# nivihelen99/NetFlow

Measured on AMD Instinct MI355X. Metric: device-resident payload GB/s checksummed, batched packets, 1/2/4/8 MI355X, higher is better.
Workload: dtype u16 one's-complement (u8 frames, u32 word sums); 1 GPU; C1: 1M x 1500 B IPv4+UDP, device-resident; packets_per_gpu=1048576, frame_align=128, frame_bytes_per_gpu=1572864000, parallelism=independent shards x1

## Files before the change

include/nfcs.h:

```cpp
#ifndef NFCS_H
#define NFCS_H

#include <stddef.h>
#include <stdint.h>

#ifdef __cplusplus
extern "C" {
#endif

#if defined(__GNUC__)
#define NFCS_API __attribute__((visibility("default")))
#else
#define NFCS_API
#endif

#define NFCS_ABI_VERSION 2


typedef struct nfcs_desc {
    uint32_t off16;
    uint32_t len;
} nfcs_desc;

typedef struct nfcs_patch {
    uint16_t ip_off;
    uint16_t l4_off;
    uint8_t ip[2];
    uint8_t l4[2];
} nfcs_patch;

#define NFCS_PATCH_NONE 0xFFFFu

enum {
    NFCS_ST_NONE = 0,
    NFCS_ST_V4 = 1,
    NFCS_ST_V4_TCP = 2,
    NFCS_ST_V4_UDP = 3,
    NFCS_ST_V4_ICMP = 4,
    NFCS_ST_V4_L4SKIP = 5,
    NFCS_ST_V6 = 6,
    NFCS_ST_V6_TCP = 7,
    NFCS_ST_V6_UDP = 8,
    NFCS_ST_V6_L4SKIP = 9,
    NFCS_ST_NO_ROUTE = 11,
    NFCS_ST_NOT_IPV4 = 12,
    NFCS_ST_TTL_EXPIRED = 13,
    NFCS_ST_OOB = 14,
    NFCS_ST_BAD_DESC = 15,
    NFCS_ST_VLAN_FAIL = 16,
    NFCS_ST_FLAG_VLAN = 0x20,
    NFCS_ST_FLAG_OVERLAP = 0x40,
    NFCS_ST_FLAG_FWD = 0x80
};

enum {
    NFCS_OK = 0,
    NFCS_EINVAL = -1,
    NFCS_EHIP = -2,
    NFCS_ENOMEM = -3,
    NFCS_ENODEV = -4
};

enum {
    NFCS_CFG_C0_64B_V4 = 0,
    NFCS_CFG_C1_1500B_UDP = 1,
    NFCS_CFG_C2_9000B_TCP = 2,
    NFCS_CFG_C3_MIXED = 3
};

typedef struct nfcs_ctx nfcs_ctx;

NFCS_API int nfcs_abi_version(void);
NFCS_API const char* nfcs_strerror(int err);
NFCS_API int nfcs_last_hip_error(void);


NFCS_API int nfcs_ctx_create(int device, nfcs_ctx** out);
NFCS_API int nfcs_ctx_destroy(nfcs_ctx* ctx);
NFCS_API void* nfcs_ctx_stream(nfcs_ctx* ctx);
NFCS_API int nfcs_ctx_set_slot_bytes(nfcs_ctx* ctx, uint32_t bytes);
NFCS_API int nfcs_ctx_launch_footprint(nfcs_ctx* ctx, uint64_t arena_bytes, const nfcs_desc* d_desc,
                                       uint32_t n, uint64_t* mean);
NFCS_API int nfcs_ctx_host_numa(nfcs_ctx* ctx, int* node, int* local);


NFCS_API int nfcs_update_device(nfcs_ctx* ctx, uint8_t* d_arena, uint64_t arena_bytes,
                                const nfcs_desc* d_desc, uint32_t n, uint8_t* d_status,
                                nfcs_patch* d_patch, void* stream);

#define NFCS_HOST_ZERO_COPY_AUTO_BYTES (32u << 20)
#define NFCS_HOST_PATCH_ONLY 1u
#define NFCS_HOST_ZERO_COPY 2u
#define NFCS_HOST_FRAMES 4u
NFCS_API int nfcs_update_host(nfcs_ctx* ctx, uint8_t* h_arena, uint64_t arena_bytes,
                              const nfcs_desc* h_desc, uint32_t n, uint8_t* h_status,
                              uint32_t flags);

#define NFCS_FRAME_RELEVANT_BYTES 131072u
NFCS_API int nfcs_update_host_frames(nfcs_ctx* ctx, uint8_t* const* frames, const uint32_t* lens, uint32_t n,
                                     uint8_t* h_status, uint32_t flags);


typedef struct nfcs_nexthop {
    uint8_t dst_mac[6];
    uint8_t src_mac[6];
} nfcs_nexthop;
#define NFCS_NH_NONE 0xFFFFFFFFu

NFCS_API int nfcs_l3_forward_device(nfcs_ctx* ctx, uint8_t* d_arena, uint64_t arena_bytes,
                                    const nfcs_desc* d_desc, const uint32_t* d_nh, uint32_t n,
                                    const nfcs_nexthop* d_table, uint32_t table_n,
                                    uint8_t* d_status, void* stream);



enum {
    NFCS_RT_FORWARD = 0,
    NFCS_RT_BAD_DESC = 1,
    NFCS_RT_NOT_IPV4 = 2,
    NFCS_RT_LOCAL = 3,
    NFCS_RT_TTL_EXPIRED = 4,
    NFCS_RT_NO_ROUTE = 5,
    NFCS_RT_ARP_MISS = 6,
    NFCS_RT_NO_IF_MAC = 7
};
#define NFCS_IF_NONE 0xFFFFFFFFu

typedef struct nfcs_fib_route {
    uint32_t network;
    uint32_t mask;
    uint32_t next_hop_ip;
    uint32_t egress_if;
} nfcs_fib_route;
typedef struct nfcs_fib_arp {
    uint32_t ip;
    uint8_t mac[6];
    uint8_t pad[2];
} nfcs_fib_arp;
typedef struct nfcs_fib_if_mac {
    uint32_t egress_if;
    uint8_t mac[6];
    uint8_t pad[2];
} nfcs_fib_if_mac;

#define NFCS_FIB_MAX_ROUTES 4096u

typedef struct nfcs_fib nfcs_fib;
NFCS_API int nfcs_fib_create(nfcs_fib** out);
NFCS_API int nfcs_fib_destroy(nfcs_fib* fib);
NFCS_API int nfcs_fib_set_routes(nfcs_fib* fib, const nfcs_fib_route* routes, uint32_t n);
NFCS_API int nfcs_fib_set_arp(nfcs_fib* fib, const nfcs_fib_arp* arp, uint32_t n);
NFCS_API int nfcs_fib_set_if_macs(nfcs_fib* fib, const nfcs_fib_if_mac* if_macs, uint32_t n);
NFCS_API int nfcs_fib_set_local_ips(nfcs_fib* fib, const uint32_t* ips, uint32_t n);
NFCS_API int nfcs_fib_commit(nfcs_fib* fib);
NFCS_API int nfcs_fib_upload(nfcs_ctx* ctx, nfcs_fib* fib);
NFCS_API int nfcs_fib_nexthops(const nfcs_fib* fib, const nfcs_nexthop** d_table, uint32_t* table_n);
NFCS_API int nfcs_fib_nexthops_host(const nfcs_fib* fib, nfcs_nexthop* out, uint32_t cap, uint32_t* table_n);
NFCS_API int nfcs_fib_lookup_host(const nfcs_fib* fib, uint32_t dst_ip, uint32_t ttl, uint32_t* verdict,
                                  uint32_t* nh, uint32_t* egress_if);

NFCS_API int nfcs_route_lookup_device(nfcs_ctx* ctx, const nfcs_fib* fib, const uint8_t* d_arena,
                                      uint64_t arena_bytes, const nfcs_desc* d_desc, uint32_t n,
                                      uint32_t* d_nh, uint32_t* d_egress_if, uint8_t* d_verdict,
                                      void* stream);

// ... 284 lines not shown
#define NFCS_ACL_LIST_NONE 0xFFFFFFFFu
#define NFCS_ACL_NO_PORT 4u
typedef struct nfcs_aclset nfcs_aclset;
NFCS_API int nfcs_aclset_create(nfcs_aclset** out);
NFCS_API int nfcs_aclset_destroy(nfcs_aclset* set);
NFCS_API int nfcs_aclset_set_list(nfcs_aclset* set, uint32_t list_id, const nfcs_acl_rule* rules, uint32_t n);
NFCS_API int nfcs_aclset_remove_list(nfcs_aclset* set, uint32_t list_id);
NFCS_API int nfcs_aclset_bind_port(nfcs_aclset* set, uint32_t port_id, uint32_t list_id);
NFCS_API int nfcs_aclset_clear(nfcs_aclset* set);
NFCS_API int nfcs_aclset_commit(nfcs_aclset* set);
NFCS_API int nfcs_aclset_upload(nfcs_ctx* ctx, nfcs_aclset* set);
NFCS_API int nfcs_aclset_info(const nfcs_aclset* set, uint32_t* ports, uint32_t* lists, uint32_t* rules_padded);
NFCS_API int nfcs_aclset_eval_host(const nfcs_aclset* set, uint32_t port, const uint8_t* frame, uint32_t len,
                                   uint32_t* action, uint32_t* rule_index, uint32_t* redirect_port);

NFCS_API int nfcs_egress_acl_device(nfcs_ctx* ctx, const nfcs_aclset* set, const uint8_t* d_arena,
                                    uint64_t arena_bytes, const nfcs_desc* d_desc, uint32_t n, uint32_t* d_port,
                                    uint8_t* d_action, uint32_t* d_rule, uint32_t* d_redirect,
                                    uint32_t* d_denied_pkts, uint64_t* d_denied_bytes, void* stream);
NFCS_API int nfcs_egress_acl_host(const nfcs_aclset* set, const uint8_t* arena, uint64_t arena_bytes,
                                  const nfcs_desc* desc, uint32_t n, uint32_t* port, uint8_t* action,
                                  uint32_t* rule, uint32_t* redirect, uint32_t* denied_pkts,
                                  uint64_t* denied_bytes);


enum { NFCS_SCHED_STRICT_PRIORITY = 0, NFCS_SCHED_WRR = 1, NFCS_SCHED_DRR = 2 };
typedef struct nfcs_txq nfcs_txq;

NFCS_API int nfcs_txq_create(nfcs_ctx* ctx, const nfcs_egress* eg, nfcs_txq** out);
NFCS_API int nfcs_txq_destroy(nfcs_txq* txq);
NFCS_API int nfcs_txq_set_scheduler(nfcs_txq* txq, uint32_t port_id, uint32_t sched);
NFCS_API int nfcs_txq_reset(nfcs_txq* txq);
NFCS_API int nfcs_txq_info(const nfcs_txq* txq, uint32_t* ports, uint32_t* keys, uint64_t* ring_slots);
NFCS_API int nfcs_txq_state_device(nfcs_txq* txq, uint32_t* head, uint8_t* last, void* stream);
NFCS_API int nfcs_txq_state_host(const nfcs_txq* txq, uint32_t* head, uint8_t* last);

NFCS_API int nfcs_txq_append_device(nfcs_ctx* ctx, nfcs_txq* txq, const uint32_t* d_order,
                                    const uint32_t* d_key_start, const uint32_t* d_depth, const uint64_t* d_handle,
                                    const nfcs_desc* d_desc, uint32_t n, void* stream);
NFCS_API int nfcs_txq_append_host(nfcs_txq* txq, const uint32_t* order, const uint32_t* key_start,
                                  const uint32_t* depth, const uint64_t* handle, const nfcs_desc* desc, uint32_t n);

NFCS_API int nfcs_txq_dequeue_device(nfcs_ctx* ctx, nfcs_txq* txq, const uint32_t* d_budget, uint32_t budget_all,
                                     uint32_t* d_depth, uint64_t* d_tx, uint32_t tx_cap, uint8_t* d_tx_queue,
                                     uint32_t* d_tx_start, uint32_t* d_dequeued, void* stream);
NFCS_API int nfcs_txq_dequeue_host(nfcs_txq* txq, const uint32_t* budget, uint32_t budget_all, uint32_t* depth,
                                   uint64_t* tx, uint32_t tx_cap, uint8_t* tx_queue, uint32_t* tx_start,
                                   uint32_t* dequeued);
NFCS_API int nfcs_txq_closed_form_host(uint32_t sched, uint32_t num_queues, uint32_t last, const uint32_t* depth,
                                       uint32_t budget, uint32_t* take, uint32_t* new_last, uint8_t* seq,
                                       uint32_t seq_cap);


typedef struct nfcs_flow_key {
    uint32_t hash;
    uint16_t vlan_id;
    uint16_t ethertype;
    uint8_t src_mac[6];
    uint8_t dst_mac[6];
    uint8_t protocol;
    uint8_t is_ipv6;
    uint16_t src_port;
    uint16_t dst_port;
    uint8_t reserved[6];
    uint8_t src_ip[16];
    uint8_t dst_ip[16];
} nfcs_flow_key;

NFCS_API int nfcs_flow_keys_device(nfcs_ctx* ctx, const uint8_t* d_arena, uint64_t arena_bytes,
                                   const nfcs_desc* d_desc, uint32_t n, nfcs_flow_key* d_keys,
                                   uint32_t* d_hash, void* stream);


NFCS_API int nfcs_shard_bytes(const nfcs_desc* h_desc, uint32_t n, uint32_t parts, uint32_t* bounds);


NFCS_API int nfcs_layout_config(int config, uint64_t seed, uint64_t first_index, uint32_t n,
                                uint32_t align, nfcs_desc* h_desc, uint64_t* arena_bytes);

NFCS_API int nfcs_gen_config_device(nfcs_ctx* ctx, int config, uint64_t seed,
                                    uint64_t first_index, uint32_t n, uint8_t* d_arena,
                                    uint64_t arena_bytes, const nfcs_desc* d_desc, void* stream);

NFCS_API int nfcs_digest_device(nfcs_ctx* ctx, const uint8_t* d_arena, uint64_t arena_bytes,
                                const nfcs_desc* d_desc, uint32_t n, uint64_t first_index,
                                uint64_t* h_digest, void* stream);

NFCS_API int nfcs_device_alloc(nfcs_ctx* ctx, size_t bytes, void** out);
NFCS_API int nfcs_device_free(nfcs_ctx* ctx, void* p);
NFCS_API int nfcs_host_alloc(nfcs_ctx* ctx, size_t bytes, void** out);
NFCS_API int nfcs_host_free(nfcs_ctx* ctx, void* p);
NFCS_API int nfcs_memcpy_h2d(nfcs_ctx* ctx, void* dst, const void* src, size_t bytes);
NFCS_API int nfcs_memcpy_d2h(nfcs_ctx* ctx, void* dst, const void* src, size_t bytes);
NFCS_API int nfcs_stream_sync(nfcs_ctx* ctx, void* stream);

NFCS_API int nfcs_time_update_device(nfcs_ctx* ctx, uint8_t* d_arena, uint64_t arena_bytes,
                                     const nfcs_desc* d_desc, uint32_t n, uint8_t* d_status,
                                     int iters, void* stream, float* ms);
NFCS_API int nfcs_time_update_batches(nfcs_ctx* ctx, uint32_t batches, uint8_t* const* d_arenas,
                                      const uint64_t* arena_bytes, const nfcs_desc* const* d_descs,
                                      uint32_t n, int iters, void* stream, float* ms);
NFCS_API int nfcs_time_flow_keys_device(nfcs_ctx* ctx, const uint8_t* d_arena, uint64_t arena_bytes,
                                        const nfcs_desc* d_desc, uint32_t n, nfcs_flow_key* d_keys,
                                        uint32_t* d_hash, int iters, void* stream, float* ms);
NFCS_API int nfcs_time_l3_forward_device(nfcs_ctx* ctx, uint8_t* d_arena, uint64_t arena_bytes,
                                         const nfcs_desc* d_desc, const uint32_t* d_nh,
                                         uint32_t n, const nfcs_nexthop* d_table, uint32_t table_n,
                                         uint8_t* d_status, int iters, void* stream, float* ms);

NFCS_API int nfcs_time_stream_read(nfcs_ctx* ctx, const uint8_t* d_buf, uint64_t bytes, int form,
                                   int iters, void* stream, float* ms);
NFCS_API int nfcs_time_frames_read(nfcs_ctx* ctx, const uint8_t* d_arena, uint64_t arena_bytes,
                                   const nfcs_desc* d_desc, uint32_t n, int iters, void* stream, float* ms);
NFCS_API int nfcs_time_vlan_device(nfcs_ctx* ctx, uint8_t* d_arena, uint64_t arena_bytes,
                                   nfcs_desc* d_desc, uint32_t n, uint32_t op_all,
                                   uint32_t op_alt, uint32_t cap_all, uint8_t* d_status, int iters,
                                   void* stream, float* ms);

#ifdef __cplusplus
}
#endif
#endif
```

netflow_amd/__init__.py:

```python
from __future__ import annotations

import ctypes
import os
import subprocess

import numpy as np

HERE = os.path.dirname(os.path.abspath(__file__))
ROOT = os.path.dirname(HERE)
LIB_PATH = os.environ.get("NFCS_LIB") or os.path.join(HERE, "libnfcs.so")
HEADER = os.path.join(ROOT, "include", "nfcs.h")
SOURCES = [os.path.join(HERE, "csrc", "nfcs_kernels.hip"), os.path.join(HERE, "csrc", "nfcs_api.hip")]

DESC_DTYPE = np.dtype([("off16", "<u4"), ("len", "<u4")])
PATCH_DTYPE = np.dtype([("ip_off", "<u2"), ("l4_off", "<u2"), ("ip", "u1", (2,)), ("l4", "u1", (2,))])

ST_NONE, ST_V4, ST_V4_TCP, ST_V4_UDP, ST_V4_ICMP, ST_V4_L4SKIP = 0, 1, 2, 3, 4, 5
ST_V6, ST_V6_TCP, ST_V6_UDP, ST_V6_L4SKIP, ST_OOB, ST_BAD_DESC = 6, 7, 8, 9, 14, 15
ST_FLAG_OVERLAP = 0x40
ST_NO_ROUTE, ST_NOT_IPV4, ST_TTL_EXPIRED, ST_FLAG_FWD = 11, 12, 13, 0x80
NH_NONE = 0xFFFFFFFF
ST_VLAN_FAIL, ST_FLAG_VLAN = 16, 0x20
VLAN_NOP, VLAN_PUSH, VLAN_POP = 0, 0x40000000, 0x80000000


def vlan_push_op(vid: int, prio: int = 0) -> int:
    return VLAN_PUSH | ((prio & 7) << 13) | (vid & 0xFFF)

RT_FORWARD, RT_BAD_DESC, RT_NOT_IPV4, RT_LOCAL, RT_TTL_EXPIRED, RT_NO_ROUTE, RT_ARP_MISS, RT_NO_IF_MAC = range(8)
IF_NONE = 0xFFFFFFFF
FIB_MAX_ROUTES = 4096
FIB_ROUTE_DTYPE = np.dtype([("network", "<u4"), ("mask", "<u4"), ("next_hop_ip", "<u4"), ("egress_if", "<u4")])
FIB_ARP_DTYPE = np.dtype([("ip", "<u4"), ("mac", "u1", (6,)), ("pad", "u1", (2,))])
FIB_IF_MAC_DTYPE = np.dtype([("egress_if", "<u4"), ("mac", "u1", (6,)), ("pad", "u1", (2,))])

ACL_PERMIT, ACL_DENY, ACL_REDIRECT, ACL_BAD_DESC = range(4)
ACL_NO_MATCH = 0xFFFFFFFF
ACL_MAX_RULES = 512
ACL_GROUP = 4
(ACL_F_SRC_MAC, ACL_F_DST_MAC, ACL_F_VLAN_ID, ACL_F_ETHERTYPE, ACL_F_SRC_IP, ACL_F_DST_IP, ACL_F_PROTOCOL,
 ACL_F_SRC_PORT, ACL_F_DST_PORT) = (1 << k for k in range(9))
ACL_RULE_DTYPE = np.dtype([("fields", "<u4"), ("rule_id", "<u4"), ("src_mac", "u1", (6,)), ("dst_mac", "u1", (6,)),
                           ("vlan_id", "<u2"), ("ethertype", "<u2"), ("src_ip", "<u4"), ("dst_ip", "<u4"),
                           ("src_ip_mask", "<u4"), ("dst_ip_mask", "<u4"), ("src_port", "<u2"), ("dst_port", "<u2"),
                           ("protocol", "u1"), ("action", "u1"), ("pad", "u1", (2,)), ("redirect_port", "<u4")])
assert ACL_RULE_DTYPE.itemsize == 52
ACL_NO_PORT = 4
ACL_LIST_NONE = 0xFFFFFFFF
ACLSET_MAX_LISTS = 128

(L2_FORWARD, L2_BAD_DESC, L2_SKIP, L2_NO_ETH, L2_FLOOD, L2_DROP_SAME_PORT, L2_DROP_LINK_DOWN, L2_DROP_STP,
 L2_DROP_VLAN) = range(9)
L2_LEARN_NONE, L2_LEARN_NEW, L2_LEARN_REFRESH, L2_LEARN_MOVED = range(4)
L2_ACCESS, L2_TRUNK, L2_HYBRID = range(3)
FDB_MAX_ENTRIES = 1 << 20
L2_MAX_PORTS = 1024
FDB_ENTRY_DTYPE = np.dtype([("mac", "u1", (6,)), ("vlan_id", "<u2"), ("port", "<u4"), ("is_static", "u1"),
                            ("pad", "u1", (3,))])
L2_PORT_DTYPE = np.dtype([("port_id", "<u4"), ("link_up", "u1"), ("stp_forwarding", "u1"), ("has_vlan_config", "u1"),
                          ("type", "u1"), ("native_vlan", "<u2"), ("pad", "<u2")])
assert FDB_ENTRY_DTYPE.itemsize == 16 and L2_PORT_DTYPE.itemsize == 12

FLOOD_TILE_PKTS = 1024
ITEM_NONE = 0xFFFFFFFF
FLOOD_TOTALS_DTYPE = np.dtype([("items", "<u4"), ("items_needed", "<u4"), ("copies", "<u4"), ("flooded", "<u4"),
                               ("copy_bytes", "<u8"), ("copy_bytes_needed", "<u8")])
assert FLOOD_TOTALS_DTYPE.itemsize == 32

ICMP_TILE_PKTS = 1024
(ICMP_ST_NONE, ICMP_ST_ECHO_REPLY, ICMP_ST_TIME_EXCEEDED, ICMP_ST_UNREACHABLE, ICMP_ST_TO_CPU, ICMP_ST_IGNORED,
 ICMP_ST_NO_LOCAL_MAC, ICMP_ST_SRC_NO_ROUTE, ICMP_ST_SRC_NO_IF_IP, ICMP_ST_SRC_ARP_MISS, ICMP_ST_SRC_NO_IF_MAC,
 ICMP_ST_PORT_DOWN, ICMP_ST_OOB, ICMP_ST_TOO_LONG, ICMP_ST_OVERFLOW) = range(15)
ICMP_LOCAL_DTYPE = np.dtype([("ip", "<u4"), ("mac", "u1", (6,)), ("pad", "u1", (2,))])
ICMP_IF_IP_DTYPE = np.dtype([("egress_if", "<u4"), ("ip", "<u4")])
ICMP_TOTALS_DTYPE = np.dtype([("messages", "<u4"), ("messages_needed", "<u4"), ("echo_replies", "<u4"),
                              ("errors", "<u4"), ("msg_bytes", "<u8"), ("msg_bytes_needed", "<u8")])
assert ICMP_LOCAL_DTYPE.itemsize == 12 and ICMP_IF_IP_DTYPE.itemsize == 8 and ICMP_TOTALS_DTYPE.itemsize == 32

QOS_MAX_QUEUES = 8
QUEUE_NONE = 0xFF
EGRESS_TILE_PKTS = 1024
EQ_ENQUEUED, EQ_SKIP, EQ_DROP_NO_CONFIG, EQ_DROP_FULL, EQ_BAD_QUEUE = range(5)
EGRESS_PORT_DTYPE = np.dtype([("port_id", "<u4"), ("has_vlan_config", "u1"), ("type", "u1"), ("tag_native", "u1"),
                              ("has_qos", "u1"), ("native_vlan", "<u2"), ("num_queues", "u1"), ("pad", "u1"),
                              ("max_queue_depth", "<u4")])
assert EGRESS_PORT_DTYPE.itemsize == 16
SCHED_STRICT_PRIORITY, SCHED_WRR, SCHED_DRR = range(3)

NEXTHOP_DTYPE = np.dtype([("dst_mac", "u1", (6,)), ("src_mac", "u1", (6,))])
FLOW_KEY_DTYPE = np.dtype([("hash", "<u4"), ("vlan_id", "<u2"), ("ethertype", "<u2"),
                           ("src_mac", "u1", (6,)), ("dst_mac", "u1", (6,)), ("protocol", "u1"),
                           ("is_ipv6", "u1"), ("src_port", "<u2"), ("dst_port", "<u2"),
                           ("reserved", "u1", (6,)), ("src_ip", "u1", (16,)), ("dst_ip", "u1", (16,))])
assert FLOW_KEY_DTYPE.itemsize == 64
CFG_C0, CFG_C1, CFG_C2, CFG_C3 = 0, 1, 2, 3
HOST_PATCH_ONLY, HOST_ZERO_COPY, HOST_FRAMES = 1, 2, 4
PATCH_NONE = 0xFFFF


class NfcsError(RuntimeError):
    pass


KERNARG_PRELOAD = ["-mllvm", "-amdgpu-kernarg-preload-count=8"]


def build(verbose: bool = False) -> str:
    out = os.path.join(HERE, "libnfcs.so")
    cmd = ["hipcc", "--offload-arch=gfx950", "-O3", "-fPIC", "-shared", "-std=c++17", *KERNARG_PRELOAD,
           "-I" + os.path.join(ROOT, "include"), "-I" + os.path.join(HERE, "csrc"), *SOURCES, "-o", out]
    if verbose:
        print(" ".join(cmd))
    subprocess.run(cmd, check=True)
    return out


ABI_VERSION = 2
_lib = None
_vp = ctypes.c_void_p
_u32 = ctypes.c_uint32
_u64 = ctypes.c_uint64


def _declare(L):
    sig = {
        "nfcs_abi_version": ([], ctypes.c_int),
        "nfcs_strerror": ([ctypes.c_int], ctypes.c_char_p),
        "nfcs_last_hip_error": ([], ctypes.c_int),
        "nfcs_ctx_create": ([ctypes.c_int, ctypes.POINTER(_vp)], ctypes.c_int),
        "nfcs_ctx_destroy": ([_vp], ctypes.c_int),
        "nfcs_ctx_stream": ([_vp], _vp),
        "nfcs_ctx_set_slot_bytes": ([_vp, ctypes.c_uint32], ctypes.c_int),
        "nfcs_ctx_launch_footprint": ([_vp, _u64, _vp, _u32, ctypes.POINTER(_u64)], ctypes.c_int),
        "nfcs_update_device": ([_vp, _vp, _u64, _vp, _u32, _vp, _vp, _vp], ctypes.c_int),
        "nfcs_update_host": ([_vp, _vp, _u64, _vp, _u32, _vp, _u32], ctypes.c_int),
        "nfcs_update_host_frames": ([_vp, _vp, _vp, _u32, _vp, _u32], ctypes.c_int),
        "nfcs_layout_config": ([ctypes.c_int, _u64, _u64, _u32, _u32, _vp, ctypes.POINTER(_u64)], ctypes.c_int),
        "nfcs_shard_bytes": ([_vp, _u32, _u32, _vp], ctypes.c_int),
        "nfcs_ctx_host_numa": ([_vp, ctypes.POINTER(ctypes.c_int), ctypes.POINTER(ctypes.c_int)], ctypes.c_int),
        "nfcs_gen_config_device": ([_vp, ctypes.c_int, _u64, _u64, _u32, _vp, _u64, _vp, _vp], ctypes.c_int),
        "nfcs_digest_device": ([_vp, _vp, _u64, _vp, _u32, _u64, ctypes.POINTER(_u64), _vp], ctypes.c_int),
        "nfcs_device_alloc": ([_vp, ctypes.c_size_t, ctypes.POINTER(_vp)], ctypes.c_int),
        "nfcs_device_free": ([_vp, _vp], ctypes.c_int),
        "nfcs_host_alloc": ([_vp, ctypes.c_size_t, ctypes.POINTER(_vp)], ctypes.c_int),
        "nfcs_host_free": ([_vp, _vp], ctypes.c_int),
        "nfcs_memcpy_h2d": ([_vp, _vp, _vp, ctypes.c_size_t], ctypes.c_int),
        "nfcs_memcpy_d2h": ([_vp, _vp, _vp, ctypes.c_size_t], ctypes.c_int),
        "nfcs_stream_sync": ([_vp, _vp], ctypes.c_int),
        "nfcs_time_update_device": ([_vp, _vp, _u64, _vp, _u32, _vp, ctypes.c_int, _vp,
                                     ctypes.POINTER(ctypes.c_float)], ctypes.c_int),
        "nfcs_time_update_batches": ([_vp, _u32, _vp, _vp, _vp, _u32, ctypes.c_int, _vp,
                                      ctypes.POINTER(ctypes.c_float)], ctypes.c_int),
        "nfcs_l3_forward_device": ([_vp, _vp, _u64, _vp, _vp, _u32, _vp, _u32, _vp, _vp],
                                   ctypes.c_int),
        "nfcs_vlan_device": ([_vp, _vp, _u64, _vp, _u32, _vp, _u32, _vp, _u32, _vp, _vp],
                             ctypes.c_int),
        "nfcs_time_vlan_device": ([_vp, _vp, _u64, _vp, _u32, _u32, _u32, _u32, _vp, ctypes.c_int,
                                   _vp, ctypes.POINTER(ctypes.c_float)], ctypes.c_int),
        "nfcs_flow_keys_device": ([_vp, _vp, _u64, _vp, _u32, _vp, _vp, _vp], ctypes.c_int),
        "nfcs_time_stream_read": ([_vp, _vp, _u64, ctypes.c_int, ctypes.c_int, _vp, _vp], ctypes.c_int),
        "nfcs_time_frames_read": ([_vp, _vp, _u64, _vp, _u32, ctypes.c_int, _vp, _vp], ctypes.c_int),
        "nfcs_time_flow_keys_device": ([_vp, _vp, _u64, _vp, _u32, _vp, _vp, ctypes.c_int, _vp,
                                        ctypes.POINTER(ctypes.c_float)], ctypes.c_int),
        "nfcs_time_l3_forward_device": ([_vp, _vp, _u64, _vp, _vp, _u32, _vp, _u32, _vp,
                                         ctypes.c_int, _vp, ctypes.POINTER(ctypes.c_float)],
                                        ctypes.c_int),
        "nfcs_fib_create": ([ctypes.POINTER(_vp)], ctypes.c_int),
        "nfcs_fib_destroy": ([_vp], ctypes.c_int),
        "nfcs_fib_set_routes": ([_vp, _vp, _u32], ctypes.c_int),
        "nfcs_fib_set_arp": ([_vp, _vp, _u32], ctypes.c_int),
        "nfcs_fib_set_if_macs": ([_vp, _vp, _u32], ctypes.c_int),
        "nfcs_fib_set_local_ips": ([_vp, _vp, _u32], ctypes.c_int),
        "nfcs_fib_commit": ([_vp], ctypes.c_int),
        "nfcs_fib_upload": ([_vp, _vp], ctypes.c_int),
        "nfcs_fib_nexthops": ([_vp, ctypes.POINTER(_vp), ctypes.POINTER(_u32)], ctypes.c_int),
        "nfcs_fib_nexthops_host": ([_vp, _vp, _u32, ctypes.POINTER(_u32)], ctypes.c_int),
        "nfcs_fib_lookup_host": ([_vp, _u32, _u32, ctypes.POINTER(_u32), ctypes.POINTER(_u32),
                                  ctypes.POINTER(_u32)], ctypes.c_int),
        "nfcs_route_lookup_device": ([_vp, _vp, _vp, _u64, _vp, _u32, _vp, _vp, _vp, _vp], ctypes.c_int),
        "nfcs_acl_create": ([ctypes.POINTER(_vp)], ctypes.c_int),
        "nfcs_acl_destroy": ([_vp], ctypes.c_int),
        "nfcs_acl_set_rules": ([_vp, _vp, _u32], ctypes.c_int),
        "nfcs_acl_commit": ([_vp], ctypes.c_int),
        "nfcs_acl_upload": ([_vp, _vp], ctypes.c_int),
        "nfcs_acl_eval_host": ([_vp, _vp, _u32, ctypes.POINTER(_u32), ctypes.POINTER(_u32),
                                ctypes.POINTER(_u32)], ctypes.c_int),
        "nfcs_acl_eval_device": ([_vp, _vp, _vp, _u64, _vp, _u32, _vp, _vp, _vp, _vp, _vp], ctypes.c_int),
        "nfcs_fdb_create": ([ctypes.POINTER(_vp)], ctypes.c_int),
        "nfcs_fdb_destroy": ([_vp], ctypes.c_int),
        "nfcs_fdb_set_entries": ([_vp, _vp, _u32], ctypes.c_int),
        "nfcs_fdb_set_port": ([_vp, _vp, _vp, _u32], ctypes.c_int),
        "nfcs_fdb_clear_ports": ([_vp], ctypes.c_int),
        "nfcs_fdb_commit": ([_vp], ctypes.c_int),
        "nfcs_fdb_upload": ([_vp, _vp], ctypes.c_int),
        "nfcs_fdb_stats": ([_vp] + [ctypes.POINTER(_u32)] * 4, ctypes.c_int),
        "nfcs_fdb_lookup_host": ([_vp, _u32, _vp, _u32] + [ctypes.POINTER(_u32)] * 4, ctypes.c_int),
        "nfcs_fdb_flood_ports_host": ([_vp, _u32, _u32, _u32, _vp, _u32, ctypes.POINTER(_u32)], ctypes.c_int),
        "nfcs_l2_lookup_device": ([_vp, _vp, _u32, _vp, _u64, _vp, _u32, _vp, _vp, _vp, _vp, _vp, _vp],
                                  ctypes.c_int),
        "nfcs_flood_expand_device": ([_vp, _vp, _u32, _u32, _vp, _u64, _u64, _u32, _vp, _u32] + [_vp] * 5 + [_u32] +
                                     [_vp] * 5, ctypes.c_int),
        "nfcs_flood_expand_host": ([_vp, _u32, _u32, _u64, _u64, _u32, _vp, _u32] + [_vp] * 5 + [_u32] + [_vp] * 4,
                                   ctypes.c_int),
        "nfcs_icmp_create": ([ctypes.POINTER(_vp)], ctypes.c_int),
        "nfcs_icmp_destroy": ([_vp], ctypes.c_int),
        "nfcs_icmp_set_local": ([_vp, _vp, _u32], ctypes.c_int),
        "nfcs_icmp_set_if_ips": ([_vp, _vp, _u32], ctypes.c_int),
        "nfcs_icmp_set_ports_up": ([_vp, _vp, _u32, _u32], ctypes.c_int),
        "nfcs_icmp_commit": ([_vp], ctypes.c_int),
        "nfcs_icmp_upload": ([_vp, _vp], ctypes.c_int),
        "nfcs_fib_resolve_host": ([_vp, _u32, ctypes.POINTER(_u32), ctypes.POINTER(_u32), ctypes.POINTER(_u32)],
                                  ctypes.c_int),
        "nfcs_icmp_respond_device": ([_vp, _vp, _vp, _u32, _vp, _u64, _u64, _u32, _vp, _u32, _vp, _vp, _u32] +
                                     [_vp] * 6, ctypes.c_int),
        "nfcs_icmp_respond_host": ([_vp, _vp, _u32, _vp, _u64, _u64, _u32, _vp, _u32, _vp, _vp, _u32] + [_vp] * 5,
                                   ctypes.c_int),
        "nfcs_egress_create": ([ctypes.POINTER(_vp)], ctypes.c_int),
        "nfcs_egress_destroy": ([_vp], ctypes.c_int),
        "nfcs_egress_set_port": ([_vp, _vp], ctypes.c_int),
        "nfcs_egress_clear_ports": ([_vp], ctypes.c_int),
        "nfcs_egress_commit": ([_vp], ctypes.c_int),
        "nfcs_egress_upload": ([_vp, _vp], ctypes.c_int),
        "nfcs_egress_keys": ([_vp, ctypes.POINTER(_u32), ctypes.POINTER(_u32)], ctypes.c_int),
# ... 611 lines not shown
    cap = int(min(int(depth.sum(dtype=np.uint64)), budget)) if want_seq else 0
    seq = np.full(cap, QUEUE_NONE, np.uint8)
    _check(lib().nfcs_txq_closed_form_host(int(sched), nq, int(last), depth.ctypes.data if nq else None, int(budget),
                                           take.ctypes.data if nq else None, ctypes.byref(new_last),
                                           seq.ctypes.data if cap else None, cap), "nfcs_txq_closed_form_host")
    return take, int(new_last.value), seq if want_seq else None


class DeviceBuffer:

    def __init__(self, engine: "Engine", nbytes: int):
        self.engine = engine
        self.nbytes = int(nbytes)
        p = _vp()
        _check(lib().nfcs_device_alloc(engine.ctx, max(self.nbytes, 16), ctypes.byref(p)), "device_alloc")
        self.ptr = p.value

    def upload(self, a: np.ndarray, offset: int = 0):
        a = np.ascontiguousarray(a)
        if offset < 0 or offset + a.nbytes > self.nbytes:
            raise NfcsError(f"upload of {a.nbytes} B at {offset} past a {self.nbytes}-byte buffer")
        if a.nbytes:
            _check(lib().nfcs_memcpy_h2d(self.engine.ctx, self.ptr + offset, a.ctypes.data, a.nbytes), "h2d")
        return self

    def download(self, dtype=np.uint8, count: int | None = None, offset: int = 0) -> np.ndarray:
        dtype = np.dtype(dtype)
        count = (self.nbytes - offset) // dtype.itemsize if count is None else count
        if offset < 0 or offset + count * dtype.itemsize > self.nbytes:
            raise NfcsError(f"download of {count} x {dtype} at {offset} past a {self.nbytes}-byte buffer")
        out = np.empty(count, dtype=dtype)
        if out.nbytes:
            _check(lib().nfcs_memcpy_d2h(self.engine.ctx, out.ctypes.data, self.ptr + offset, out.nbytes), "d2h")
        return out

    def free(self):
        if self.ptr:
            lib().nfcs_device_free(self.engine.ctx, self.ptr)
            self.ptr = None

    def __del__(self):
        try:
            self.free()
        except Exception:
            pass


class Engine:

    def __init__(self, device: int = 0):
        self.device = device
        self._pinned = {}
        c = _vp()
        _check(lib().nfcs_ctx_create(device, ctypes.byref(c)), f"nfcs_ctx_create({device})")
        self.ctx = c.value

    def close(self):
        if getattr(self, "ctx", None):
            for p in list(self._pinned):
                lib().nfcs_host_free(self.ctx, p)
            self._pinned.clear()
            lib().nfcs_ctx_destroy(self.ctx)
            self.ctx = None

    def __enter__(self):
        return self

    def __exit__(self, *a):
        self.close()

    @property
    def stream(self) -> int:
        return lib().nfcs_ctx_stream(self.ctx)

    def set_slot_bytes(self, nbytes: int):
        _check(lib().nfcs_ctx_set_slot_bytes(self.ctx, int(nbytes)), "set_slot_bytes")

    def launch_footprint(self, arena_bytes: int, desc, n: int) -> int:
        m = _u64()
        p = desc.ptr if isinstance(desc, DeviceBuffer) else int(desc)
        _check(lib().nfcs_ctx_launch_footprint(self.ctx, arena_bytes, p, n, ctypes.byref(m)), "launch_footprint")
        return int(m.value)

    def host_numa(self) -> tuple[int, bool]:
        node, local = ctypes.c_int(), ctypes.c_int()
        _check(lib().nfcs_ctx_host_numa(self.ctx, ctypes.byref(node), ctypes.byref(local)), "host_numa")
        return node.value, bool(local.value)

    def alloc(self, nbytes: int) -> DeviceBuffer:
        return DeviceBuffer(self, nbytes)

    def host_array(self, nbytes: int) -> np.ndarray:
        p = _vp()
        size = max(int(nbytes), 16)
        _check(lib().nfcs_host_alloc(self.ctx, size, ctypes.byref(p)), "host_alloc")
        self._pinned[p.value] = size
        return np.ctypeslib.as_array((ctypes.c_uint8 * size).from_address(p.value))[:nbytes]

    def host_free(self, arr: np.ndarray):
        p = arr.__array_interface__["data"][0]
        if self._pinned.pop(p, None) is None:
            raise NfcsError("host_free: not a live host_array of this engine")
        _check(lib().nfcs_host_free(self.ctx, p), "host_free")

    def sync(self, stream=None):
        _check(lib().nfcs_stream_sync(self.ctx, stream), "stream_sync")

    def update_device(self, arena: DeviceBuffer | int, arena_bytes: int, desc: DeviceBuffer | int,
                      n: int, status=None, patch=None, stream=None):
        ptr = lambda b: None if b is None else (b.ptr if isinstance(b, DeviceBuffer) else int(b))
        _check(lib().nfcs_update_device(self.ctx, ptr(arena), arena_bytes, ptr(desc), n,
                                        ptr(status), ptr(patch), stream), "nfcs_update_device")

    def update_host(self, arena: np.ndarray, desc: np.ndarray, want_status: bool = True,
                    mode: str = "patch") -> np.ndarray | None:
        flags = {"patch": 0, "frames": HOST_FRAMES, "zero_copy": HOST_ZERO_COPY}[mode]
        assert arena.dtype == np.uint8 and arena.flags.c_contiguous
        desc = np.ascontiguousarray(desc, dtype=DESC_DTYPE)
        n = len(desc)
        status = np.zeros(n, dtype=np.uint8) if want_status else None
        _check(lib().nfcs_update_host(self.ctx, arena.ctypes.data, arena.nbytes,
                                      desc.ctypes.data if n else None, n,
                                      status.ctypes.data if want_status and n else None,
                                      flags), "nfcs_update_host")
        return status

    def update_host_frames(self, buf: np.ndarray, offsets: np.ndarray, lens: np.ndarray,
                           want_status: bool = True) -> np.ndarray | None:
        assert buf.dtype == np.uint8 and buf.flags.c_contiguous
        offsets = np.asarray(offsets, dtype=np.int64)
        lens = np.ascontiguousarray(lens, dtype=np.uint32)
        n = len(lens)
        assert len(offsets) == n and (n == 0 or int((offsets + lens.astype(np.int64)).max()) <= buf.nbytes)
        ptrs = np.where(offsets < 0, 0, np.uint64(buf.ctypes.data) + offsets.astype(np.uint64)).astype(np.uint64)
        status = np.zeros(n, dtype=np.uint8) if want_status else None
        _check(lib().nfcs_update_host_frames(self.ctx, ptrs.ctypes.data if n else None,
                                             lens.ctypes.data if n else None, n,
                                             status.ctypes.data if want_status and n else None, 0),
               "nfcs_update_host_frames")
        return status

    def l3_forward_device(self, arena, arena_bytes: int, desc, nh, n: int, table, table_n: int,
                          status=None, stream=None):
        ptr = lambda b: None if b is None else (b.ptr if isinstance(b, DeviceBuffer) else int(b))
        _check(lib().nfcs_l3_forward_device(self.ctx, ptr(arena), arena_bytes, ptr(desc), ptr(nh), n,
                                            ptr(table), table_n, ptr(status), stream),
               "nfcs_l3_forward_device")

    def route_lookup_device(self, fib: Fib, arena, arena_bytes: int, desc, n: int, nh, egress_if=None,
                            verdict=None, stream=None):
        ptr = lambda b: None if b is None else (b.ptr if isinstance(b, DeviceBuffer) else int(b))
        _check(lib().nfcs_route_lookup_device(self.ctx, fib.ptr, ptr(arena), arena_bytes, ptr(desc), n, ptr(nh),
                                              ptr(egress_if), ptr(verdict), stream), "nfcs_route_lookup_device")

    def acl_eval_device(self, acl: Acl, arena, arena_bytes: int, desc, n: int, action, rule=None, redirect=None,
                        nh=None, stream=None):
        ptr = lambda b: None if b is None else (b.ptr if isinstance(b, DeviceBuffer) else int(b))
        _check(lib().nfcs_acl_eval_device(self.ctx, acl.ptr, ptr(arena), arena_bytes, ptr(desc), n, ptr(action),
                                          ptr(rule), ptr(redirect), ptr(nh), stream), "nfcs_acl_eval_device")

    def l2_lookup_device(self, fdb: "Fdb", ingress_port: int, arena, arena_bytes: int, desc, n: int, egress_port,
                         rt_verdict=None, verdict=None, vlan=None, learn=None, stream=None):
        ptr = lambda b: None if b is None else (b.ptr if isinstance(b, DeviceBuffer) else int(b))
        _check(lib().nfcs_l2_lookup_device(self.ctx, fdb.ptr, int(ingress_port), ptr(arena), arena_bytes, ptr(desc), n,
                                           ptr(rt_verdict), ptr(egress_port), ptr(verdict), ptr(vlan), ptr(learn),
                                           stream), "nfcs_l2_lookup_device")
# ... 49 lines not shown
        ptr = lambda b: None if b is None else (b.ptr if isinstance(b, DeviceBuffer) else int(b))
        _check(lib().nfcs_txq_dequeue_device(self.ctx, txq.ptr, ptr(budget), int(budget_all), ptr(depth), ptr(tx),
                                             int(tx_cap), ptr(tx_queue), ptr(tx_start), ptr(dequeued), stream),
               "nfcs_txq_dequeue_device")

    def vlan_device(self, arena, arena_bytes: int, desc, n: int, ops=None, op_all: int = 0,
                    caps=None, cap_all: int = 0, status=None, stream=None):
        ptr = lambda b: None if b is None else (b.ptr if isinstance(b, DeviceBuffer) else int(b))
        _check(lib().nfcs_vlan_device(self.ctx, ptr(arena), arena_bytes, ptr(desc), n, ptr(ops),
                                      op_all, ptr(caps), cap_all, ptr(status), stream),
               "nfcs_vlan_device")

    def time_vlan_device(self, arena, arena_bytes, desc, n, op_all, op_alt, cap_all, iters,
                         status=None, stream=None) -> float:
        ms = ctypes.c_float()
        ptr = lambda b: None if b is None else (b.ptr if isinstance(b, DeviceBuffer) else int(b))
        _check(lib().nfcs_time_vlan_device(self.ctx, ptr(arena), arena_bytes, ptr(desc), n, op_all,
                                           op_alt, cap_all, ptr(status), iters, stream,
                                           ctypes.byref(ms)), "time_vlan_device")
        return float(ms.value)

    def flow_keys_device(self, arena, arena_bytes: int, desc, n: int, keys=None, hashes=None,
                         stream=None):
        ptr = lambda b: None if b is None else (b.ptr if isinstance(b, DeviceBuffer) else int(b))
        _check(lib().nfcs_flow_keys_device(self.ctx, ptr(arena), arena_bytes, ptr(desc), n, ptr(keys),
                                           ptr(hashes), stream), "nfcs_flow_keys_device")

    def time_flow_keys_device(self, arena, arena_bytes, desc, n, keys, hashes, iters,
                              stream=None) -> float:
        ms = ctypes.c_float()
        ptr = lambda b: None if b is None else (b.ptr if isinstance(b, DeviceBuffer) else int(b))
        _check(lib().nfcs_time_flow_keys_device(self.ctx, ptr(arena), arena_bytes, ptr(desc), n,
                                                ptr(keys), ptr(hashes), iters, stream,
                                                ctypes.byref(ms)), "time_flow_keys_device")
        return float(ms.value)

    def time_stream_read(self, buf, nbytes, iters, form=0, stream=None) -> float:
        ms = ctypes.c_float()
        p = buf.ptr if isinstance(buf, DeviceBuffer) else int(buf)
        _check(lib().nfcs_time_stream_read(self.ctx, p, nbytes & ~15, form, iters, stream,
                                           ctypes.byref(ms)), "time_stream_read")
        return float(ms.value)

    def time_frames_read(self, arena, arena_bytes, desc, n, iters, stream=None) -> float:
        ms = ctypes.c_float()
        p = lambda b: b.ptr if isinstance(b, DeviceBuffer) else int(b)
        _check(lib().nfcs_time_frames_read(self.ctx, p(arena), arena_bytes, p(desc), n, iters, stream,
                                           ctypes.byref(ms)), "time_frames_read")
        return float(ms.value)

    def time_l3_forward_device(self, arena, arena_bytes, desc, nh, n, table, table_n, iters,
                               status=None, stream=None) -> float:
        ms = ctypes.c_float()
        ptr = lambda b: None if b is None else (b.ptr if isinstance(b, DeviceBuffer) else int(b))
        _check(lib().nfcs_time_l3_forward_device(self.ctx, ptr(arena), arena_bytes, ptr(desc),
                                                 ptr(nh), n, ptr(table), table_n, ptr(status),
                                                 iters, stream, ctypes.byref(ms)),
               "time_l3_forward_device")
        return float(ms.value)

    def time_update_device(self, arena, arena_bytes, desc, n, iters, status=None, stream=None) -> float:
        ms = ctypes.c_float()
        _check(lib().nfcs_time_update_device(self.ctx, arena.ptr, arena_bytes, desc.ptr, n,
                                             None if status is None else status.ptr, iters, stream,
                                             ctypes.byref(ms)), "time_update_device")
        return float(ms.value)

    def time_update_batches(self, batches, n, iters, stream=None) -> float:
        k = len(batches)
        p = lambda b: b.ptr if isinstance(b, DeviceBuffer) else int(b)
        arenas = (_vp * k)(*[p(a) for a, _, _ in batches])
        sizes = (_u64 * k)(*[int(nb) for _, nb, _ in batches])
        descs = (_vp * k)(*[p(d) for _, _, d in batches])
        ms = ctypes.c_float()
        _check(lib().nfcs_time_update_batches(self.ctx, k, arenas, sizes, descs, n, iters, stream,
                                              ctypes.byref(ms)), "time_update_batches")
        return float(ms.value)

    def gen_config_device(self, config: int, seed: int, first: int, n: int,
                          arena: DeviceBuffer, arena_bytes: int, desc: DeviceBuffer, stream=None):
        _check(lib().nfcs_gen_config_device(self.ctx, config, seed, first, n, arena.ptr, arena_bytes,
                                            desc.ptr, stream), "gen_config_device")

    def digest_device(self, arena: DeviceBuffer, arena_bytes: int, desc: DeviceBuffer, n: int,
                      first: int = 0, stream=None) -> int:
        out = _u64()
        _check(lib().nfcs_digest_device(self.ctx, arena.ptr, arena_bytes, desc.ptr, n, first,
                                        ctypes.byref(out), stream), "digest_device")
        return int(out.value)

    def config_batch(self, config: int, seed: int, first: int, n: int, align: int = 16):
        hdesc, nbytes = layout_config(config, seed, first, n, align)
        d_desc = self.alloc(max(hdesc.nbytes, 16)).upload(hdesc)
        d_arena = self.alloc(max(nbytes, 16))
        self.gen_config_device(config, seed, first, n, d_arena, nbytes, d_desc)
        self.sync()
        return d_arena, nbytes, d_desc, hdesc
```

netflow_amd/csrc/nfcs_api.hip:

```cpp
#include <pthread.h>
#include <sched.h>
#include <stdio.h>
#include <stdlib.h>
#include <string.h>
#include <sys/mman.h>
#include <sys/syscall.h>
#include <unistd.h>

#include <algorithm>
#include <chrono>
#include <condition_variable>
#include <mutex>
#include <new>
#include <thread>
#include <vector>

#include "nfcs_internal.h"

struct HostBlock {
    void* p = nullptr;
    size_t bytes = 0;
    bool mapped = false;
};

class Workers {
public:
    ~Workers() { stop(); }
    void start(int n, const cpu_set_t* cpus) noexcept {
        for (int i = 0; i < n; ++i) {
            try {
                th_.emplace_back([this, cpus] { loop(cpus); });
            } catch (...) {
                break;
            }
        }
    }
    void stop() noexcept {
        {
            std::lock_guard<std::mutex> l(mu_);
            quit_ = true;
        }
        cv_.notify_all();
        for (auto& t : th_) t.join();
        th_.clear();
        quit_ = false;
    }
    int size() const { return (int)th_.size(); }
    template <class F>
    void run(int k, const F& fn) noexcept {
        if (k <= 1 || th_.empty()) {
            for (int i = 0; i < k; ++i) fn(i);
            return;
        }
        run_erased(k, [](const void* f, int i) { (*(const F*)f)(i); }, &fn);
    }

private:
    void run_erased(int k, void (*call)(const void*, int), const void* fn) noexcept {
        std::unique_lock<std::mutex> l(mu_);
        call_ = call;
        job_ = fn;
        parts_ = k;
        next_ = 0;
        pending_ = k;
        ++gen_;
        cv_.notify_all();
        take(l);
        done_.wait(l, [&] { return pending_ == 0; });
        job_ = nullptr;
    }
    void take(std::unique_lock<std::mutex>& l) {
        while (next_ < parts_) {
            const int i = next_++;
            void (*const call)(const void*, int) = call_;
            const void* const f = job_;
            l.unlock();
            call(f, i);
            l.lock();
            if (--pending_ == 0) done_.notify_all();
        }
    }
    void loop(const cpu_set_t* cpus) {
        if (cpus) (void)pthread_setaffinity_np(pthread_self(), sizeof(cpu_set_t), cpus);
        std::unique_lock<std::mutex> l(mu_);
        uint64_t seen = 0;
        for (;;) {
            cv_.wait(l, [&] { return quit_ || (gen_ != seen && next_ < parts_); });
            if (quit_) return;
            take(l);
            seen = gen_;
        }
    }
    std::vector<std::thread> th_;
    std::mutex mu_;
    std::condition_variable cv_, done_;
    void (*call_)(const void*, int) = nullptr;
    const void* job_ = nullptr;
    int parts_ = 0, next_ = 0, pending_ = 0;
    uint64_t gen_ = 0;
    bool quit_ = false;
};

struct nfcs_ctx {
    nfcs::DevInfo di;
    int numa_node = -1;
    bool numa_local = false;
    bool have_cpus = false;
    cpu_set_t node_cpus;
    HostBlock hb[2];
    hipStream_t stream = nullptr;
    static constexpr int kSlots = 2;
    static constexpr size_t kStageBytes = size_t(64) << 20;
    bool host_ready = false;
    hipStream_t hs[kSlots] = {nullptr, nullptr};
    hipEvent_t done[kSlots] = {nullptr, nullptr};
    hipEvent_t staged[kSlots] = {nullptr, nullptr};
    size_t stage_bytes = 0;
    uint32_t stage_pkts = 0;
    int copy_threads = 8;
    Workers workers;
    uint8_t* d_arena[kSlots] = {nullptr, nullptr};
    nfcs_desc* d_desc[kSlots] = {nullptr, nullptr};
    uint8_t* d_status[kSlots] = {nullptr, nullptr};
    nfcs_patch* d_patch[kSlots] = {nullptr, nullptr};
    uint64_t* done_host = nullptr;
    uint64_t* done_dev = nullptr;
    uint64_t* done_ctr = nullptr;
    uint64_t done_base[kSlots] = {0, 0};
    int slot_wait[kSlots] = {0, 0};
    uint8_t* z_block[kSlots] = {nullptr, nullptr};
    uint8_t* h_arena[kSlots] = {nullptr, nullptr};
    nfcs_desc* h_desc[kSlots] = {nullptr, nullptr};
    uint8_t* h_status[kSlots] = {nullptr, nullptr};
    nfcs_patch* h_patch[kSlots] = {nullptr, nullptr};
    uint64_t* d_digest = nullptr;
    hipEvent_t ev0 = nullptr, ev1 = nullptr;
    nfcs_patch* ws = nullptr;
    size_t ws_cap = 0;
    hipEvent_t ws_ev = nullptr;
    hipStream_t ws_stream = nullptr;
    bool ws_used = false;
    bool ws_own = false;
    uint32_t* eq_ws = nullptr;
    uint64_t eq_cap = 0;
    hipEvent_t eq_ev = nullptr;
    hipStream_t eq_stream = nullptr;
    bool eq_used = false;
    bool eq_own = false;
    uint32_t slot_bytes = 0;
    static constexpr int kObsSlots = 8;
    uint64_t* obs_host = nullptr;
    uint64_t* obs_dev = nullptr;
    struct ObsBurst { const void* desc; uint32_t n; uint64_t bytes; uint32_t gen; uint64_t used; };
    ObsBurst obs_burst[kObsSlots] = {};
    uint32_t obs_gen = 0;
    uint64_t obs_clock = 0;
};

namespace {

thread_local int g_last_hip = 0;

hipError_t wait_ws_user(nfcs_ctx* c, hipStream_t st) {
    if (c->ws_own) {
        hipError_t e = hipEventRecord(c->ws_ev, c->stream);
        if (e != hipSuccess) return e;
    }
    return st ? hipStreamWaitEvent(st, c->ws_ev, 0) : hipEventSynchronize(c->ws_ev);
}

hipError_t acquire_ws(nfcs_ctx* c, size_t n, hipStream_t st) {
    if (n > c->ws_cap) {
        if (c->ws_used) {
            hipError_t e = wait_ws_user(c, nullptr);
            if (e != hipSuccess) return e;
        }
        if (c->ws) (void)hipFree(c->ws);
        c->ws = nullptr;
        c->ws_cap = 0;
        c->ws_used = false;
        const size_t cap = n < (1u << 20) ? (1u << 20) : n;
        hipError_t e = hipMalloc(&c->ws, cap * sizeof(nfcs_patch));
        if (e != hipSuccess) return e;
        c->ws_cap = cap;
    } else if (c->ws_used && c->ws_stream != st) {
        hipError_t e = wait_ws_user(c, st);
        if (e != hipSuccess) return e;
    }
    return hipSuccess;
}
hipError_t release_ws(nfcs_ctx* c, hipStream_t st) {
    c->ws_stream = st;
    c->ws_used = true;
    c->ws_own = st == c->stream;
    return c->ws_own ? hipSuccess : hipEventRecord(c->ws_ev, st);
}

hipError_t wait_eq_user(nfcs_ctx* c, hipStream_t st) {
    if (c->eq_own) {
        hipError_t e = hipEventRecord(c->eq_ev, c->stream);
        if (e != hipSuccess) return e;
    }
    return st ? hipStreamWaitEvent(st, c->eq_ev, 0) : hipEventSynchronize(c->eq_ev);
}
hipError_t acquire_eq(nfcs_ctx* c, uint64_t words, hipStream_t st) {
    if (words > c->eq_cap) {
        if (c->eq_used) {
            hipError_t e = wait_eq_user(c, nullptr);
            if (e != hipSuccess) return e;
        }
        if (c->eq_ws) (void)hipFree(c->eq_ws);
        c->eq_ws = nullptr;
        c->eq_cap = 0;
        c->eq_used = false;
        const uint64_t cap = words < (1u << 18) ? (1u << 18) : words;
        if (cap > (uint64_t)SIZE_MAX / sizeof(uint32_t)) return hipErrorOutOfMemory;
        hipError_t e = hipMalloc(&c->eq_ws, (size_t)cap * sizeof(uint32_t));
        if (e != hipSuccess) {
            c->eq_ws = nullptr;
            (void)hipGetLastError();
            return hipErrorOutOfMemory;
        }
        c->eq_cap = cap;
    } else if (c->eq_used && c->eq_stream != st) {
        hipError_t e = wait_eq_user(c, st);
        if (e != hipSuccess) return e;
    }
    return hipSuccess;
}
hipError_t release_eq(nfcs_ctx* c, hipStream_t st) {
    c->eq_stream = st;
    c->eq_used = true;
    c->eq_own = st == c->stream;
    return c->eq_own ? hipSuccess : hipEventRecord(c->eq_ev, st);
}

int hip_fail(hipError_t e) {
    g_last_hip = (int)e;
    return NFCS_EHIP;
// ... 377 lines not shown
        } else {
            event_wait(c, s);
            e = hipMemcpyAsync(c->d_desc[s], c->h_desc[s], (size_t)m * sizeof(nfcs_desc),
                               hipMemcpyHostToDevice, st);
            if (e == hipSuccess)
                e = nfcs::launch_update(c->di, d_arena, arena_bytes, c->d_desc[s], m, 0u,
                                        h_status ? c->d_status[s] : nullptr, nullptr, nullptr,
                                        nfcs::kUpdateInline, st, shape);
            if (e == hipSuccess && h_status)
                e = hipMemcpyAsync(c->h_status[s], c->d_status[s], m, hipMemcpyDeviceToHost, st);
        }
        if (e == hipSuccess) e = hipEventRecord(c->done[s], st);
        if (e != hipSuccess) {
            (void)hipStreamSynchronize(st);
            break;
        }
        first[s] = i;
        cnt[s] = m;
        i += m;
    }
    finish(s);
    finish(s ^ 1);
    if (e != hipSuccess) return hip_fail(e);
    return NFCS_OK;
}

struct Shape { uint64_t mean; nfcs::ObsReq obs; uint32_t bits = 0; };
int find_burst(const nfcs_ctx* c, uint64_t arena_bytes, const nfcs_desc* d_desc, uint32_t n) {
    for (int k = 0; k < nfcs_ctx::kObsSlots; ++k) {
        const nfcs_ctx::ObsBurst& b = c->obs_burst[k];
        if (b.gen && b.desc == d_desc && b.n == n && b.bytes == arena_bytes) return k;
    }
    return -1;
}
bool sampled_estimate(uint64_t est, bool mid = false) {
    return mid || est >= nfcs::kSmallMeanBytes || est < nfcs::kTinyMeanBytes;
}
struct ShapeRule { uint64_t mix_mean; bool ring_rows8; bool bimodal_rows8; bool packed_rows8; };
constexpr ShapeRule kUpdateRule = {nfcs::kTinyMixMeanBytes, true, false, false};
constexpr ShapeRule kFwdRule = {nfcs::kTinyMixMeanBytes, true, true, true};
constexpr ShapeRule kVlanRule = {nfcs::kVlanMixMeanBytes, false, false, false};
Shape peek_shape(const nfcs_ctx* c, uint64_t arena_bytes, const nfcs_desc* d_desc, uint32_t n, int* slot,
                 const ShapeRule& rule = kUpdateRule) {
    *slot = -1;
    if (c->slot_bytes) return {c->slot_bytes, {}};
    if (n == 0) return {arena_bytes, {}};
    const uint64_t est = arena_bytes / n;
    if (!sampled_estimate(est, rule.packed_rows8) || !c->obs_host) return {est, {}};
    const int k = find_burst(c, arena_bytes, d_desc, n);
    if (k < 0) return {est, {}};
    *slot = k;
    const uint64_t o = __atomic_load_n(c->obs_host + k, __ATOMIC_RELAXED);
    const uint32_t gen = c->obs_burst[k].gen;
    const nfcs::ObsReq req = {c->obs_dev + k, ((uint64_t)gen << 32) | n};
    if ((uint32_t)(o >> 32) != gen || !((uint32_t)o & nfcs::kObsPresent)) return {est, req};
    uint64_t mean = std::min<uint64_t>((uint32_t)o & nfcs::kObsMeanMask, est);
    const bool bimodal = rule.bimodal_rows8 && (((uint32_t)o >> nfcs::kObsMidShift) & 7u) < nfcs::kObsMidMin8;
    if (mean < nfcs::kTinyMeanBytes && mean >= rule.mix_mean && !bimodal &&
        (((uint32_t)o >> nfcs::kObsLongShift) & 0x1FFu) > nfcs::kTinyLongMax)
        mean = nfcs::kTinyMeanBytes;
    const uint32_t bits = (uint32_t)o & (nfcs::kObsUnaligned | nfcs::kObsMixed);
    if (rule.ring_rows8 && !bits && (est >= nfcs::kSmallMeanBytes || rule.packed_rows8) &&
        mean >= nfcs::kTinyMeanBytes && mean < nfcs::kSmallMeanBytes)
        mean = nfcs::kTinyMeanBytes - 1;
    return {mean, req, bits};
}
Shape launch_shape(nfcs_ctx* c, uint64_t arena_bytes, const nfcs_desc* d_desc, uint32_t n,
                   const ShapeRule& rule = kUpdateRule) {
    int k = -1;
    Shape sh = peek_shape(c, arena_bytes, d_desc, n, &k, rule);
    if (sh.obs.slot == nullptr && k < 0 && !c->slot_bytes && n && c->obs_host &&
        sampled_estimate(arena_bytes / n, rule.packed_rows8)) {
        k = 0;
        for (int j = 1; j < nfcs_ctx::kObsSlots; ++j)
            if (c->obs_burst[j].used < c->obs_burst[k].used) k = j;
        if (++c->obs_gen == 0) c->obs_gen = 1;
        c->obs_burst[k] = {d_desc, n, arena_bytes, c->obs_gen, 0};
        sh.obs = {c->obs_dev + k, ((uint64_t)c->obs_gen << 32) | n};
    }
    if (k >= 0) c->obs_burst[k].used = ++c->obs_clock;
    return sh;
}

int update_device(nfcs_ctx* c, uint8_t* d_arena, uint64_t arena_bytes, const nfcs_desc* d_desc,
                  uint32_t n, uint8_t* d_status, nfcs_patch* d_patch, hipStream_t st) {
    if (!d_patch) NFCS_HIP(acquire_ws(c, n, st));
    const Shape sh = launch_shape(c, arena_bytes, d_desc, n);
    NFCS_HIP(nfcs::launch_update(c->di, d_arena, arena_bytes, d_desc, n, 0u, d_status, d_patch,
                                 d_patch ? nullptr : c->ws, nfcs::kUpdateAuto, st, sh.mean, sh.obs));
    if (!d_patch) NFCS_HIP(release_ws(c, st));
    return NFCS_OK;
}

int l3_forward_device(nfcs_ctx* c, uint8_t* d_arena, uint64_t arena_bytes, const nfcs_desc* d_desc,
                      const uint32_t* d_nh, uint32_t n, const nfcs_nexthop* d_table, uint32_t table_n,
                      uint8_t* d_status, hipStream_t st) {
    const bool dfr = n > nfcs::kFwdDeferAbovePackets;
    if (dfr) NFCS_HIP(acquire_ws(c, nfcs::kSubBatchPackets, st));
    const Shape sh = launch_shape(c, arena_bytes, d_desc, n, kFwdRule);
    NFCS_HIP(nfcs::launch_l3_forward(c->di, d_arena, arena_bytes, d_desc, d_nh, n, d_table, table_n,
                                     d_status, dfr ? c->ws : nullptr, st, sh.mean, sh.obs));
    if (dfr) NFCS_HIP(release_ws(c, st));
    return NFCS_OK;
}

}

extern "C" {

NFCS_API int nfcs_abi_version(void) { return NFCS_ABI_VERSION; }

NFCS_API const char* nfcs_strerror(int err) {
    switch (err) {
    case NFCS_OK: return "ok";
    case NFCS_EINVAL: return "invalid argument";
    case NFCS_EHIP: return "HIP runtime error";
    case NFCS_ENOMEM: return "out of memory";
    case NFCS_ENODEV: return "no gfx950 device";
    default: return "unknown error";
    }
}

NFCS_API int nfcs_last_hip_error(void) { return g_last_hip; }

NFCS_API int nfcs_ctx_create(int device, nfcs_ctx** out) {
    if (!out) return NFCS_EINVAL;
    *out = nullptr;
    int ndev = 0;
    if (hipGetDeviceCount(&ndev) != hipSuccess || device < 0 || device >= ndev) {
        (void)hipGetLastError();
        return NFCS_ENODEV;
    }
    DeviceGuard dg_(device);
    if (dg_.err != hipSuccess) return hip_fail(dg_.err);
    hipDeviceProp_t prop;
    NFCS_HIP(hipGetDeviceProperties(&prop, device));
    if (strncmp(prop.gcnArchName, "gfx950", 6) != 0) return NFCS_ENODEV;
    nfcs_ctx* c = new (std::nothrow) nfcs_ctx();
    if (!c) return NFCS_ENOMEM;
    c->di.device = device;
    c->di.cus = prop.multiProcessorCount;
    strncpy(c->di.arch, prop.gcnArchName, sizeof(c->di.arch) - 1);
    hipError_t e = hipStreamCreateWithFlags(&c->stream, hipStreamNonBlocking);
    if (e == hipSuccess) e = hipMalloc(&c->d_digest, sizeof(uint64_t));
    if (e == hipSuccess) e = hipEventCreateWithFlags(&c->ws_ev, hipEventDisableTiming);
    if (e == hipSuccess) e = hipEventCreateWithFlags(&c->eq_ev, hipEventDisableTiming);
    if (e == hipSuccess) e = hipEventCreate(&c->ev0);
    if (e == hipSuccess) e = hipEventCreate(&c->ev1);
    if (e == hipSuccess) e = hipHostMalloc((void**)&c->obs_host, nfcs_ctx::kObsSlots * sizeof(uint64_t), hipHostMallocMapped);
    if (e == hipSuccess) {
        for (int k = 0; k < nfcs_ctx::kObsSlots; ++k) c->obs_host[k] = 0;
        e = hipHostGetDevicePointer((void**)&c->obs_dev, c->obs_host, 0);
    }
    if (e != hipSuccess) {
        nfcs_ctx_destroy(c);
        return hip_fail(e);
    }
    *out = c;
    return NFCS_OK;
}

NFCS_API int nfcs_ctx_destroy(nfcs_ctx* c) {
    if (!c) return NFCS_OK;
    DeviceGuard dg_(c->di.device);
    if (c->stream) (void)hipStreamSynchronize(c->stream);
    if (c->ws_used && !c->ws_own && c->ws_ev) (void)hipEventSynchronize(c->ws_ev);
    if (c->eq_used && !c->eq_own && c->eq_ev) (void)hipEventSynchronize(c->eq_ev);
    free_host_pipeline(c);
    if (c->d_digest) (void)hipFree(c->d_digest);
    if (c->eq_ws) (void)hipFree(c->eq_ws);
    if (c->eq_ev) (void)hipEventDestroy(c->eq_ev);
    if (c->ws) (void)hipFree(c->ws);
    if (c->ws_ev) (void)hipEventDestroy(c->ws_ev);
    if (c->ev0) (void)hipEventDestroy(c->ev0);
    if (c->ev1) (void)hipEventDestroy(c->ev1);
    if (c->stream) (void)hipStreamDestroy(c->stream);
    if (c->obs_host) (void)hipHostFree(c->obs_host);
    delete c;
    return NFCS_OK;
}

NFCS_API void* nfcs_ctx_stream(nfcs_ctx* c) { return c ? (void*)c->stream : nullptr; }

NFCS_API int nfcs_ctx_set_slot_bytes(nfcs_ctx* c, uint32_t bytes) {
    if (!c) return NFCS_EINVAL;
    c->slot_bytes = bytes;
    return NFCS_OK;
}

NFCS_API int nfcs_ctx_launch_footprint(nfcs_ctx* c, uint64_t arena_bytes, const nfcs_desc* d_desc,
                                       uint32_t n, uint64_t* mean) {
    if (!c || !mean) return NFCS_EINVAL;
    int slot = -1;
    *mean = peek_shape(c, arena_bytes, d_desc, n, &slot).mean;
    return NFCS_OK;
}

NFCS_API int nfcs_ctx_host_numa(nfcs_ctx* c, int* node, int* local) {
    if (!c || !node || !local) return NFCS_EINVAL;
    DeviceGuard dg_(c->di.device);
    if (dg_.err != hipSuccess) return hip_fail(dg_.err);
    const int rc = ensure_host_pipeline(c);
    if (rc) return rc;
    *node = c->numa_node;
    *local = c->numa_local ? 1 : 0;
    return NFCS_OK;
}

NFCS_API int nfcs_update_device(nfcs_ctx* c, uint8_t* d_arena, uint64_t arena_bytes,
                                const nfcs_desc* d_desc, uint32_t n, uint8_t* d_status,
                                nfcs_patch* d_patch, void* stream) {
    if (!c) return NFCS_EINVAL;
    DeviceGuard dg_(c->di.device);
    if (dg_.err != hipSuccess) return hip_fail(dg_.err);
    if (n == 0) return NFCS_OK;
    if (!d_arena || !d_desc || ((uintptr_t)d_arena & 15u)) return NFCS_EINVAL;
    return update_device(c, d_arena, arena_bytes, d_desc, n, d_status, d_patch, pick(c, stream));
}

NFCS_API int nfcs_l3_forward_device(nfcs_ctx* c, uint8_t* d_arena, uint64_t arena_bytes,
                                    const nfcs_desc* d_desc, const uint32_t* d_nh, uint32_t n,
                                    const nfcs_nexthop* d_table, uint32_t table_n,
                                    uint8_t* d_status, void* stream) {
    if (!c) return NFCS_EINVAL;
    DeviceGuard dg_(c->di.device);
    if (dg_.err != hipSuccess) return hip_fail(dg_.err);
    if (n == 0) return NFCS_OK;
    if (!d_arena || !d_desc || !d_nh || ((uintptr_t)d_arena & 15u)) return NFCS_EINVAL;
    if (table_n > 0 && (!d_table || ((uintptr_t)d_table & 3u))) return NFCS_EINVAL;
    return l3_forward_device(c, d_arena, arena_bytes, d_desc, d_nh, n, d_table, table_n, d_status,
                             pick(c, stream));
}

NFCS_API int nfcs_vlan_device(nfcs_ctx* c, uint8_t* d_arena, uint64_t arena_bytes,
                              nfcs_desc* d_desc, uint32_t n, const uint32_t* d_ops,
                              uint32_t op_all, const uint32_t* d_caps, uint32_t cap_all,
                              uint8_t* d_status, void* stream) {
    if (!c) return NFCS_EINVAL;
    DeviceGuard dg_(c->di.device);
    if (dg_.err != hipSuccess) return hip_fail(dg_.err);
    if (n == 0) return NFCS_OK;
    if (!d_arena || !d_desc || ((uintptr_t)d_arena & 15u)) return NFCS_EINVAL;
    if (((uintptr_t)d_ops & 3u) || ((uintptr_t)d_caps & 3u)) return NFCS_EINVAL;
    const Shape sh = launch_shape(c, arena_bytes, d_desc, n, kVlanRule);
    NFCS_HIP(nfcs::launch_vlan(c->di, d_arena, arena_bytes, d_desc, n, d_ops, op_all, d_caps,
                               cap_all, d_status, pick(c, stream), sh.mean, sh.obs, sh.bits));
    return NFCS_OK;
}

NFCS_API int nfcs_flow_keys_device(nfcs_ctx* c, const uint8_t* d_arena, uint64_t arena_bytes,
                                   const nfcs_desc* d_desc, uint32_t n, nfcs_flow_key* d_keys,
                                   uint32_t* d_hash, void* stream) {
    if (!c) return NFCS_EINVAL;
    DeviceGuard dg_(c->di.device);
    if (dg_.err != hipSuccess) return hip_fail(dg_.err);
    if (n == 0) return NFCS_OK;
    if (!d_arena || !d_desc || ((uintptr_t)d_arena & 15u) || ((uintptr_t)d_keys & 15u))
        return NFCS_EINVAL;
    NFCS_HIP(nfcs::launch_flow_keys(c->di, d_arena, arena_bytes, d_desc, n, d_keys, d_hash,
                                    pick(c, stream)));
    return NFCS_OK;
}

}

struct nfcs_fib {
    nfcs::FibInputs in;
    nfcs::FibTables t;
    bool committed = false;
// ... 1494 lines not shown
            }
            nt_fence();
        });
        finish(s);
        if (e != hipSuccess) break;
        hipStream_t st = c->hs[s];
        if (c->z_block[s] && bytes <= kDirectChunkBytes) {
            e = nfcs::launch_update(c->di, zdev(c, s, dst), bytes ? bytes : 16, zdev(c, s, hd), m, 0u,
                                    h_status ? zdev(c, s, c->h_status[s]) : nullptr, zdev(c, s, c->h_patch[s]),
                                    nullptr, nfcs::kUpdateRecords, st, 0, {}, done_req(c, s));
            if (e == hipSuccess) e = hipEventRecord(c->staged[s], st);
        } else {
            event_wait(c, s);
            e = hipMemcpyAsync(c->d_desc[s], hd, (size_t)m * sizeof(nfcs_desc), hipMemcpyHostToDevice, st);
            if (e == hipSuccess && bytes) e = hipMemcpyAsync(c->d_arena[s], dst, bytes, hipMemcpyHostToDevice, st);
            if (e == hipSuccess) e = hipEventRecord(c->staged[s], st);
            if (e == hipSuccess)
                e = nfcs::launch_update(c->di, c->d_arena[s], bytes ? bytes : 16, c->d_desc[s], m, 0u, c->d_status[s],
                                        c->d_patch[s], nullptr, nfcs::kUpdateRecords, st);
            if (e == hipSuccess)
                e = hipMemcpyAsync(c->h_patch[s], c->d_patch[s], (size_t)m * sizeof(nfcs_patch), hipMemcpyDeviceToHost, st);
            if (e == hipSuccess && h_status) e = hipMemcpyAsync(c->h_status[s], c->d_status[s], m, hipMemcpyDeviceToHost, st);
        }
        if (e == hipSuccess) e = hipEventRecord(c->done[s], st);
        if (e != hipSuccess) {
            (void)hipStreamSynchronize(st);
            break;
        }
        slot[s] = {i, i1, true};
        i = i1;
        s ^= 1;
    }
    finish(s);
    finish(s ^ 1);
    if (e != hipSuccess) return hip_fail(e);
    return NFCS_OK;
}

NFCS_API int nfcs_shard_bytes(const nfcs_desc* h_desc, uint32_t n, uint32_t parts, uint32_t* bounds) {
    if (!bounds || parts == 0 || (n && !h_desc)) return NFCS_EINVAL;
    uint64_t total = 0;
    for (uint32_t i = 0; i < n; ++i) total += h_desc[i].len;
    uint32_t i = 0;
    uint64_t run = 0;
    bounds[0] = 0;
    for (uint32_t p = 1; p < parts; ++p) {
        const unsigned __int128 t = (unsigned __int128)total * p;
        const uint64_t target = (uint64_t)(t / parts) + (t % parts != 0);
        while (i < n && run < target) run += h_desc[i++].len;
        bounds[p] = i;
    }
    bounds[parts] = n;
    return NFCS_OK;
}

NFCS_API int nfcs_layout_config(int config, uint64_t seed, uint64_t first_index, uint32_t n,
                                uint32_t align, nfcs_desc* h_desc, uint64_t* arena_bytes) {
    if (config < 0 || config > 3 || align < 16 || (align & 15u)) return NFCS_EINVAL;
    uint64_t off = 0;
    for (uint32_t i = 0; i < n; ++i) {
        const uint32_t len = nfcs::config_len(config, seed, first_index + i);
        if ((off >> 4) > 0xFFFFFFFFull) return NFCS_EINVAL;
        if (h_desc) h_desc[i] = nfcs_desc{(uint32_t)(off >> 4), len};
        off += ((uint64_t)len + align - 1) / align * align;
    }
    if (arena_bytes) *arena_bytes = off;
    return NFCS_OK;
}

NFCS_API int nfcs_gen_config_device(nfcs_ctx* c, int config, uint64_t seed, uint64_t first,
                                    uint32_t n, uint8_t* d_arena, uint64_t arena_bytes,
                                    const nfcs_desc* d_desc, void* stream) {
    if (!c || config < 0 || config > 3) return NFCS_EINVAL;
    DeviceGuard dg_(c->di.device);
    if (dg_.err != hipSuccess) return hip_fail(dg_.err);
    if (n == 0) return NFCS_OK;
    if (!d_arena || !d_desc) return NFCS_EINVAL;
    NFCS_HIP(hipMemsetAsync(d_arena, 0, arena_bytes, pick(c, stream)));
    NFCS_HIP(nfcs::launch_gen_config(c->di, config, seed, first, n, d_arena, arena_bytes, d_desc,
                                     pick(c, stream)));
    return NFCS_OK;
}

NFCS_API int nfcs_digest_device(nfcs_ctx* c, const uint8_t* d_arena, uint64_t arena_bytes,
                                const nfcs_desc* d_desc, uint32_t n, uint64_t first,
                                uint64_t* h_digest, void* stream) {
    if (!c || !h_digest) return NFCS_EINVAL;
    DeviceGuard dg_(c->di.device);
    if (dg_.err != hipSuccess) return hip_fail(dg_.err);
    hipStream_t st = pick(c, stream);
    NFCS_HIP(hipMemsetAsync(c->d_digest, 0, sizeof(uint64_t), st));
    if (n) {
        if (!d_arena || !d_desc) return NFCS_EINVAL;
        NFCS_HIP(nfcs::launch_digest(c->di, d_arena, arena_bytes, d_desc, n, first, c->d_digest, st));
    }
    NFCS_HIP(hipMemcpyAsync(h_digest, c->d_digest, sizeof(uint64_t), hipMemcpyDeviceToHost, st));
    NFCS_HIP(hipStreamSynchronize(st));
    return NFCS_OK;
}

NFCS_API int nfcs_device_alloc(nfcs_ctx* c, size_t bytes, void** out) {
    if (!c || !out) return NFCS_EINVAL;
    DeviceGuard dg_(c->di.device);
    if (dg_.err != hipSuccess) return hip_fail(dg_.err);
    hipError_t e = hipMalloc(out, bytes ? bytes : 16);
    if (e == hipErrorOutOfMemory) { (void)hipGetLastError(); return NFCS_ENOMEM; }
    NFCS_HIP(e);
    return NFCS_OK;
}
NFCS_API int nfcs_device_free(nfcs_ctx* c, void* p) {
    if (!c) return NFCS_EINVAL;
    DeviceGuard dg_(c->di.device);
    if (dg_.err != hipSuccess) return hip_fail(dg_.err);
    NFCS_HIP(hipFree(p));
    return NFCS_OK;
}
NFCS_API int nfcs_host_alloc(nfcs_ctx* c, size_t bytes, void** out) {
    if (!c || !out) return NFCS_EINVAL;
    DeviceGuard dg_(c->di.device);
    if (dg_.err != hipSuccess) return hip_fail(dg_.err);
    hipError_t e = hipHostMalloc(out, bytes ? bytes : 16, hipHostMallocDefault);
    if (e == hipErrorOutOfMemory) { (void)hipGetLastError(); return NFCS_ENOMEM; }
    NFCS_HIP(e);
    return NFCS_OK;
}
NFCS_API int nfcs_host_free(nfcs_ctx* c, void* p) {
    if (!c) return NFCS_EINVAL;
    DeviceGuard dg_(c->di.device);
    if (dg_.err != hipSuccess) return hip_fail(dg_.err);
    NFCS_HIP(hipHostFree(p));
    return NFCS_OK;
}
NFCS_API int nfcs_memcpy_h2d(nfcs_ctx* c, void* dst, const void* src, size_t bytes) {
    if (!c) return NFCS_EINVAL;
    DeviceGuard dg_(c->di.device);
    if (dg_.err != hipSuccess) return hip_fail(dg_.err);
    NFCS_HIP(hipMemcpyAsync(dst, src, bytes, hipMemcpyHostToDevice, c->stream));
    NFCS_HIP(hipStreamSynchronize(c->stream));
    return NFCS_OK;
}
NFCS_API int nfcs_memcpy_d2h(nfcs_ctx* c, void* dst, const void* src, size_t bytes) {
    if (!c) return NFCS_EINVAL;
    DeviceGuard dg_(c->di.device);
    if (dg_.err != hipSuccess) return hip_fail(dg_.err);
    NFCS_HIP(hipMemcpyAsync(dst, src, bytes, hipMemcpyDeviceToHost, c->stream));
    NFCS_HIP(hipStreamSynchronize(c->stream));
    return NFCS_OK;
}
NFCS_API int nfcs_stream_sync(nfcs_ctx* c, void* stream) {
    if (!c) return NFCS_EINVAL;
    DeviceGuard dg_(c->di.device);
    if (dg_.err != hipSuccess) return hip_fail(dg_.err);
    NFCS_HIP(hipStreamSynchronize(pick(c, stream)));
    return NFCS_OK;
}


NFCS_API int nfcs_time_update_device(nfcs_ctx* c, uint8_t* d_arena, uint64_t arena_bytes,
                                     const nfcs_desc* d_desc, uint32_t n, uint8_t* d_status,
                                     int iters, void* stream, float* ms) {
    if (!c || !ms || iters <= 0) return NFCS_EINVAL;
    DeviceGuard dg_(c->di.device);
    if (dg_.err != hipSuccess) return hip_fail(dg_.err);
    hipStream_t st = pick(c, stream);
    if (!d_arena || !d_desc || ((uintptr_t)d_arena & 15u)) return NFCS_EINVAL;
    NFCS_HIP(hipEventRecord(c->ev0, st));
// ... 121 lines not shown
```

netflow_amd/csrc/nfcs_internal.h:

```cpp
#pragma once

#include <hip/hip_runtime.h>
#include <stdint.h>

#include "nfcs.h"
#include "nfcs_acl.h"
#include "nfcs_aclset.h"
#include "nfcs_egress.h"
#include "nfcs_fdb.h"
#include "nfcs_fib.h"
#include "nfcs_icmp.h"
#include "nfcs_txq.h"

namespace nfcs {

constexpr int kWave = 64;
constexpr int kWavesPerBlock = 4;
constexpr int kBlock = kWave * kWavesPerBlock;

struct DevInfo {
    int device = 0;
    int cus = 256;
    char arch[64] = {0};
};

enum : int {
    kUpdateAuto = 0,
    kUpdateRecords = 1,
    kUpdateInline = 2
};

constexpr uint32_t kDeferMeanBytes = 1280;
constexpr uint32_t kInlineMaxPackets = 65536;
constexpr uint32_t kFrameRelevantBytes = NFCS_FRAME_RELEVANT_BYTES;
constexpr uint32_t kSubBatchPackets = 1u << 19;
constexpr uint32_t kSubBatchAbovePackets = 1u << 19;
constexpr uint32_t kFwdDeferAbovePackets = kInlineMaxPackets;
constexpr uint64_t kSmallMeanBytes = 1200;
constexpr uint64_t kTinyMeanBytes = 800;
constexpr uint32_t kTinyRowBytes = 768;
constexpr uint32_t kTinyLongMax = 32;
constexpr uint64_t kTinyMixMeanBytes = 512;
constexpr uint32_t kObsPresent = 0x80000000u;
constexpr uint32_t kObsLongShift = 20;
constexpr uint32_t kObsMeanMask = 0x1FFFFu;
constexpr uint32_t kObsMidShift = 17;
constexpr uint32_t kObsMidMin8 = 2;
constexpr uint32_t kObsUnaligned = 1u << 29;
constexpr uint32_t kObsMixed = 1u << 30;
constexpr uint32_t kObsUnalignedMax = 32;
constexpr uint64_t kVlanWtMeanBytes = 256;
constexpr uint64_t kVlanMixMeanBytes = 640;
constexpr unsigned kRowsLdsPad = 30720;
constexpr unsigned kRowsLdsPad6 = 24576;

inline uint64_t shape_mean(uint64_t arena_bytes, uint32_t n, uint64_t slot_bytes) {
    return slot_bytes ? slot_bytes : arena_bytes / n;
}

struct ObsReq {
    uint64_t* slot = nullptr;
    uint64_t tag = 0;
};

struct DoneReq {
    uint64_t* flag = nullptr;
    uint64_t* ctr = nullptr;
    uint64_t base = 0;
};

hipError_t launch_update(const DevInfo& di, uint8_t* arena, uint64_t arena_bytes,
                         const nfcs_desc* desc, uint32_t n, uint32_t base16, uint8_t* status,
                         nfcs_patch* patch, nfcs_patch* ws, int form, hipStream_t stream,
                         uint64_t slot_bytes = 0, ObsReq obs = {}, DoneReq done = {});

hipError_t launch_l3_forward(const DevInfo& di, uint8_t* arena, uint64_t arena_bytes,
                             const nfcs_desc* desc, const uint32_t* nh, uint32_t n,
                             const nfcs_nexthop* table, uint32_t table_n, uint8_t* status,
                             nfcs_patch* ws, hipStream_t stream, uint64_t slot_bytes = 0,
                             ObsReq obs = {});

hipError_t launch_vlan(const DevInfo& di, uint8_t* arena, uint64_t arena_bytes, nfcs_desc* desc,
                       uint32_t n, const uint32_t* ops, uint32_t op_all, const uint32_t* caps,
                       uint32_t cap_all, uint8_t* status, hipStream_t stream, uint64_t slot_bytes = 0,
                       ObsReq obs = {}, uint32_t sample_bits = 0);

hipError_t launch_flow_keys(const DevInfo& di, const uint8_t* arena, uint64_t arena_bytes,
                            const nfcs_desc* desc, uint32_t n, nfcs_flow_key* keys,
                            uint32_t* hashes, hipStream_t stream);

struct FibDev {
    const uint2* rt_nm = nullptr;
    const uint2* rt_info = nullptr;
    uint32_t routes = 0, routes_padded = 0;
    const uint32_t* arp_ip = nullptr;
    const uint32_t* arp_nh = nullptr;
    uint32_t arps = 0;
    const uint32_t* local_ip = nullptr;
    uint32_t locals = 0;
};

hipError_t launch_route_lookup(const DevInfo& di, const FibDev& fib, const uint8_t* arena, uint64_t arena_bytes,
                               const nfcs_desc* desc, uint32_t n, uint32_t* nh, uint32_t* egress_if,
                               uint8_t* verdict, hipStream_t stream);

struct AclDev {
    const uint4* rec = nullptr;
    const uint2* act = nullptr;
    uint32_t rules = 0, rules_padded = 0;
};

hipError_t launch_acl_eval(const DevInfo& di, const AclDev& acl, const uint8_t* arena, uint64_t arena_bytes,
                           const nfcs_desc* desc, uint32_t n, uint8_t* action, uint32_t* rule, uint32_t* redirect,
                           uint32_t* nh, hipStream_t stream);

struct AclSetDev {
    const uint4* rec = nullptr;
    const uint2* act = nullptr;
    const uint2* bind = nullptr;
    uint32_t ports = 0, rules_padded = 0;
};

hipError_t launch_egress_acl(const DevInfo& di, const AclSetDev& set, const uint8_t* arena, uint64_t arena_bytes,
                             const nfcs_desc* desc, uint32_t n, uint32_t* port, uint8_t* action, uint32_t* rule,
                             uint32_t* redirect, uint32_t* denied_pkts, uint64_t* denied_bytes, hipStream_t stream);

struct FdbDev {
    const uint4* slots = nullptr;
    uint32_t slot_mask = 0, max_probe = 0;
    const uint8_t* port_state = nullptr;
    const uint16_t* port_native = nullptr;
    const uint32_t* port_vlans = nullptr;
    uint32_t ports = 0;
    const uint32_t* vlan_ports = nullptr;
    uint32_t port_words = 0;
};

hipError_t launch_l2_lookup(const DevInfo& di, const FdbDev& fdb, uint32_t ingress, const uint8_t* arena,
                            uint64_t arena_bytes, const nfcs_desc* desc, uint32_t n, const uint8_t* rt_verdict,
                            uint32_t* egress_port, uint8_t* verdict, uint16_t* vlan, uint8_t* learn,
                            hipStream_t stream);

struct EgressDev {
    const uint4* recs = nullptr;
    uint32_t ports = 0, keys = 0;
};

hipError_t launch_egress_plan(const DevInfo& di, const EgressDev& eg, const uint8_t* arena, uint64_t arena_bytes,
                              const nfcs_desc* desc, uint32_t n, const uint32_t* l3_port, const uint8_t* fwd_status,
                              const uint32_t* l2_port, uint32_t* port, uint32_t* ops, uint8_t* queue,
                              hipStream_t stream);

constexpr uint32_t kEgTile = NFCS_EGRESS_TILE_PKTS;
static_assert(kEgTile % 64u == 0 && kEgTile >= 64u, "a tile is whole rounds of one wave");
inline uint64_t egress_scratch_words(uint32_t n, uint32_t keys) {
    const uint64_t tiles = ((uint64_t)n + kEgTile - 1u) / kEgTile;
    return tiles * keys + 2ull * keys;
}
hipError_t launch_egress_enqueue(const DevInfo& di, const EgressDev& eg, const uint32_t* port, const uint8_t* queue,
                                 uint32_t n, uint32_t* depth, uint8_t* result, uint32_t* order, uint32_t* key_start,
                                 uint32_t* key_dropped, uint32_t* scratch, hipStream_t stream);

struct TxqDev {
    const uint4* port = nullptr;
    const uint64_t* ring_base = nullptr;
    uint64_t* ring = nullptr;
    uint32_t* head = nullptr;
    uint32_t* last = nullptr;
    uint32_t* take = nullptr;
    uint32_t* elem_start = nullptr;
    uint32_t* tx_start = nullptr;
    uint32_t* new_last = nullptr;
    uint32_t ports = 0, keys = 0;
    uint64_t ring_slots = 0;
};
constexpr uint32_t kTxqPlanThreads = NFCS_L2_MAX_PORTS;
static_assert(kTxqPlanThreads == 1024u, "the plan is one workgroup of 16 waves");

hipError_t launch_txq_append(const TxqDev& t, const uint32_t* order, const uint32_t* key_start, const uint32_t* depth,
                             const uint64_t* handle, const nfcs_desc* desc, uint32_t n, hipStream_t stream);
hipError_t launch_txq_dequeue(const TxqDev& t, const uint32_t* budget, uint32_t budget_all, uint32_t* depth,
                              uint64_t* tx, uint32_t tx_cap, uint8_t* tx_queue, uint32_t* tx_start, uint32_t* dequeued,
                              hipStream_t stream);

constexpr uint32_t kFloodTile = NFCS_FLOOD_TILE_PKTS;
static_assert(kFloodTile == 1024u, "a tile is one workgroup of 16 waves, one lane per packet");
struct alignas(8) FloodSum {
    uint32_t items, copies, flooded, pad;
    uint64_t bytes;
};
static_assert(sizeof(FloodSum) == 24, "six scratch words per tile");
inline uint64_t flood_scratch_words(uint32_t n) {
    const uint64_t tiles = ((uint64_t)n + kFloodTile - 1u) / kFloodTile;
    return (tiles + 1u) * (sizeof(FloodSum) / sizeof(uint32_t));
}
struct FloodArgs {
    uint8_t* arena;
    uint64_t arena_bytes, copy_base;
    uint32_t copy_align, ingress, num_ports, n, cap;
    const nfcs_desc* desc;
    const uint32_t* l3_port;
    const uint8_t* fwd_status;
    const uint32_t* l2_port;
    const uint8_t* l2_verdict;
    const uint16_t* l2_vlan;
    nfcs_desc* item_desc;
    uint32_t* item_port;
    uint32_t* item_src;
    nfcs_flood_totals* totals;
};
hipError_t launch_flood_expand(const DevInfo& di, const FdbDev& fdb, const FloodArgs& a, uint32_t* scratch,
                               hipStream_t stream);

constexpr uint32_t kIcmpTile = NFCS_ICMP_TILE_PKTS;
static_assert(kIcmpTile == kFloodTile, "the scan and its scratch are the flood stage's");
struct IcmpArgs {
    uint8_t* arena;
    uint64_t arena_bytes, msg_base;
    uint32_t msg_align, ingress, n, cap;
    const nfcs_desc* desc;
    const uint8_t* rt_verdict;
    const uint16_t* ip_id;
    nfcs_desc* msg_desc;
    uint32_t* msg_port;
    uint32_t* msg_src;
    uint8_t* status;
    nfcs_icmp_totals* totals;
};
hipError_t launch_icmp_respond(const DevInfo& di, const IcmpView& icmp, const FibView& fib, const IcmpArgs& a,
                               uint32_t* scratch, hipStream_t stream);

hipError_t launch_gen_config(const DevInfo& di, int config, uint64_t seed, uint64_t first,
                             uint32_t n, uint8_t* arena, uint64_t arena_bytes,
                             const nfcs_desc* desc, hipStream_t stream);

hipError_t launch_digest(const DevInfo& di, const uint8_t* arena, uint64_t arena_bytes,
                         const nfcs_desc* desc, uint32_t n, uint64_t first, uint64_t* d_out,
                         hipStream_t stream);

hipError_t launch_stream_read(const uint8_t* buf, uint64_t bytes, int form, unsigned long long* sink,
                              hipStream_t stream);

hipError_t launch_frames_read(const uint8_t* arena, uint64_t arena_bytes, const nfcs_desc* desc, uint32_t n,
                              unsigned long long* sink, hipStream_t stream);

uint32_t config_len(int config, uint64_t seed, uint64_t index);

}
```

netflow_amd/csrc/nfcs_kernels.hip:

```cpp
#include "nfcs_internal.h"

namespace nfcs {

#define DEV __device__ __forceinline__

DEV uint32_t rfl(uint32_t v) { return (uint32_t)__builtin_amdgcn_readfirstlane((int)v); }

DEV uint32_t xcd_block_n(uint32_t nblocks) {
    const uint32_t b = blockIdx.x, g8 = nblocks / 8u;
    return b < 8u * g8 ? (b % 8u) * g8 + b / 8u : b;
}
DEV uint32_t xcd_block() { return xcd_block_n(gridDim.x); }
DEV uint32_t bswap16(uint32_t x) { return ((x & 0xFFu) << 8) | ((x >> 8) & 0xFFu); }

__device__ __attribute__((aligned(4096))) uint4 g_zero_line[8];

DEV uint32_t comp(const uint4& v, uint32_t j) {
    const uint32_t m0 = 0u - (uint32_t)(j == 0), m1 = 0u - (uint32_t)(j == 1);
    const uint32_t m2 = 0u - (uint32_t)(j == 2), m3 = 0u - (uint32_t)(j == 3);
    return (v.x & m0) | (v.y & m1) | (v.z & m2) | (v.w & m3);
}


DEV uint4 put_byte(const uint4& v, uint32_t i, uint32_t b) {
// ... 461 lines not shown
        *p = v;
    }
}

template <int P>
struct DescW { uint32_t w[2 * P]; };

template <int P>
DEV DescW<P> load_descw(const nfcs_desc* __restrict__ desc, uint64_t pw, uint32_t n) {
    DescW<P> D;
    if (pw + P <= n) {
        const uint32_t* q = (const uint32_t*)(desc + pw);
#pragma unroll
        for (int i = 0; i < 2 * P; ++i) D.w[i] = q[i];
    } else {
#pragma unroll
        for (int i = 0; i < P; ++i) {
            const bool ok = pw + i < n;
            D.w[2 * i] = ok ? desc[pw + i].off16 : 0u;
            D.w[2 * i + 1] = ok ? desc[pw + i].len : 0u;
        }
    }
    return D;
}

template <int P>
DEV nfcs_desc pick_desc(const DescW<P>& D, uint32_t row) {
    nfcs_desc d;
    d.off16 = 0;
    d.len = 0;
#pragma unroll
    for (int i = 0; i < P; ++i) {
        const uint32_t m = 0u - (uint32_t)(row == (uint32_t)i);
        d.off16 |= D.w[2 * i] & m;
        d.len |= D.w[2 * i + 1] & m;
    }
    return d;
}

struct WaveBuf {
    __amdgpu_buffer_rsrc_t rs;
    uint32_t lo16;
    bool ok;
};
constexpr uint32_t kBufSpan16 = (1u << 28) - (1u << 13);
constexpr uint32_t kBufOob = 0xFFFFFFF0u;

template <int P>
DEV WaveBuf wave_buf(const DescW<P>& D, uint64_t pw, uint32_t n, uint8_t* arena, uint32_t base16) {
    uint32_t lo = D.w[0], hi = D.w[0];
#pragma unroll
    for (int i = 1; i < P; ++i) {
        const uint32_t o = (pw + (uint64_t)i < n) ? D.w[2 * i] : D.w[0];
        lo = min(lo, o);
        hi = max(hi, o);
    }
    lo = rfl(lo);
    hi = rfl(hi);
    WaveBuf b;
    b.lo16 = lo;
    b.ok = hi - lo < kBufSpan16;
    b.rs = __builtin_amdgcn_make_buffer_rsrc(arena + ((int64_t)lo - (int64_t)base16) * 16, (short)0, kBufOob,
                                             0x00020000);
    return b;
}

template <int K>
struct RowStage {
    uint4 v[K];
    uint8_t* frame;
    uint32_t len;
    uint32_t p;
    uint32_t valid, bad;
    uint32_t nh;
    uint32_t mis;
};

struct FwdArgs {
    const uint32_t* nh;
    const nfcs_nexthop* table;
    uint32_t table_n;
    ObsReq obs;
    DoneReq done = {};
};

DEV void signal_done(const DoneReq& d, uint32_t nblocks) {
    __builtin_amdgcn_fence(__ATOMIC_RELEASE, "");
    __syncthreads();
    if (threadIdx.x == 0) {
        const uint64_t now = __hip_atomic_fetch_add(d.ctr, 1ull, __ATOMIC_ACQ_REL, __HIP_MEMORY_SCOPE_AGENT) + 1ull;
        if (now == d.base + nblocks) {
            __builtin_amdgcn_fence(__ATOMIC_ACQUIRE, "");
            __hip_atomic_store(d.flag, now, __ATOMIC_RELEASE, __HIP_MEMORY_SCOPE_SYSTEM);
        }
    }
}

DEV void sample_footprint(const nfcs_desc* __restrict__ desc, uint64_t tag, uint32_t lane, uint64_t* obs) {
    const uint32_t n = (uint32_t)tag;
    uint32_t s = 0, c = 0, u = 0, md = 0, lo = 0xFFFFFFFFu, hi = 0;
#pragma unroll
    for (uint32_t k = 0; k < 4; ++k) {
        const nfcs_desc d = desc[(uint32_t)(((uint64_t)(4u * lane + k) * n) >> 8)];
        const uint32_t r = ((d.len < 0xFFFFu ? d.len : 0xFFFFu) + 127u) & ~127u;
        s += r;
        c += d.len > kTinyRowBytes ? 1u : 0u;
        u += (d.off16 & 7u) ? 1u : 0u;
        md += (r > 128u && r <= 1408u) ? 1u : 0u;
        lo = min(lo, r);
        hi = max(hi, r);
    }
    s = row_sum<16>(s);
    c = row_sum<16>(c);
    u = row_sum<16>(u);
    md = row_sum<16>(md);
#pragma unroll
    for (int m = 1; m < 64; m <<= 1) {
        lo = min(lo, (uint32_t)__shfl_xor((int)lo, m));
        hi = max(hi, (uint32_t)__shfl_xor((int)hi, m));
    }
    auto wave_total = [](uint32_t v) {
        return (uint32_t)__builtin_amdgcn_readlane((int)v, 0) + (uint32_t)__builtin_amdgcn_readlane((int)v, 16) +
               (uint32_t)__builtin_amdgcn_readlane((int)v, 32) + (uint32_t)__builtin_amdgcn_readlane((int)v, 48);
    };
    const uint32_t t = wave_total(s), l = wave_total(c), un = wave_total(u), mid = wave_total(md) >> 5;
    const uint32_t bits = (un > kObsUnalignedMax ? kObsUnaligned : 0u) | (hi - lo > 128u ? kObsMixed : 0u) |
                          ((mid < 7u ? mid : 7u) << kObsMidShift);
    if (lane == 0)
        __hip_atomic_store(obs, (tag & 0xFFFFFFFF00000000ull) | kObsPresent | bits | (l << kObsLongShift) | (t >> 8),
                           __ATOMIC_RELAXED, __HIP_MEMORY_SCOPE_SYSTEM);
}

template <int K, int R = 16, bool FWD = false, bool LA = false, bool BUF = false>
DEV void row_stage(RowStage<K>& S, uint8_t* arena, uint64_t arena_bytes, const nfcs_desc& d,
                   uint64_t p64, uint32_t n, uint32_t base16, uint32_t rl, const WaveBuf& wb, uint32_t nh = 0) {
    const bool valid = p64 < n;
    const uint64_t off = ((uint64_t)d.off16 - base16) * 16u;
    const bool bad = valid && ((d.off16 < base16) ||
                               (off + (((uint64_t)d.len + 15u) & ~15ull) > arena_bytes));
    const bool live = valid && !bad;
    S.valid = valid;
    S.bad = bad;
    S.p = (uint32_t)p64;
    S.len = live ? d.len : 0u;
    S.frame = arena + (live ? off : 0);
    S.mis = LA && live ? (uint32_t)(((uintptr_t)S.frame >> 4) & 7u) : 0u;
    const uint32_t nch = (S.len + 15u) >> 4;
    const uint4* src = (const uint4*)S.frame;
    if (FWD) S.nh = nh;
    if (BUF && wb.ok) {
        const uint32_t rel = (d.off16 - wb.lo16) * 16u;
#pragma unroll
        for (int k = 0; k < K; ++k) {
            const uint32_t c = rl + (uint32_t)R * k - S.mis;
            const uint32_t vo = (c < nch) ? rel + 16u * c : kBufOob;
            const u32x4_t t = k == 0 ? __builtin_amdgcn_raw_buffer_load_b128(wb.rs, vo, 0, 0)
                                     : __builtin_amdgcn_raw_buffer_load_b128(wb.rs, vo, 0, kCpolNt);
            S.v[k] = make_uint4(t.x, t.y, t.z, t.w);
        }
    } else {
#pragma unroll
        for (int k = 0; k < K; ++k) {
            const uint32_t c = rl + (uint32_t)R * k - S.mis;
            const uint4* a = (c < nch) ? src + c : g_zero_line;
            S.v[k] = k == 0 ? ld16<0>(a) : ld16<1>(a);
        }
    }
    if (FWD) __builtin_amdgcn_sched_barrier(0);
}

enum : int { SF_INLINE = 0, SF_DEFER = 1, SF_RECORDS = 2 };
constexpr uint32_t kFwdNoIp = 0xFEu, kFwdNone = 0xFFu;
DEV uint2 fwd_record(uint32_t ipw, uint32_t l4w, uint32_t ttl_new, uint32_t proto, bool tagged) {
    const bool ip = (ipw & 0xFFFFu) != NFCS_PATCH_NONE, l4 = (l4w & 0xFFFFu) != NFCS_PATCH_NONE;
    const uint32_t ipo = ip ? (ipw & 0xFFu) : kFwdNoIp, l4o = l4 ? (l4w & 0xFFu) : kFwdNone;
    const uint32_t y = (ip ? (ipw >> 16) : (tagged ? 26u : 22u)) | (l4w & 0xFFFF0000u);
    return make_uint2(ipo | ((ttl_new & 0xFFu) << 8) | ((proto & 0xFFu) << 16) | (l4o << 24), y);
}

DEV bool defer_group(uint32_t lensum, uint32_t P) { return lensum >= P * (uint32_t)kDeferMeanBytes; }
DEV uint32_t defer_len(uint32_t len) { return len < 0xFFFFu ? len : 0xFFFFu; }

template <int K, int R>
DEV uint4 hdr_view(const RowStage<K>& S, uint32_t rowbase4, uint32_t rl) {
    const uint32_t a = rl + S.mis;
    const int sl = (int)(rowbase4 + (a & (R - 1)) * 4u);
    const uint4 v0 = S.v[0], v1 = S.v[1];
    const uint4 r0 = make_uint4((uint32_t)__builtin_amdgcn_ds_bpermute(sl, (int)v0.x),
                                (uint32_t)__builtin_amdgcn_ds_bpermute(sl, (int)v0.y),
                                (uint32_t)__builtin_amdgcn_ds_bpermute(sl, (int)v0.z),
                                (uint32_t)__builtin_amdgcn_ds_bpermute(sl, (int)v0.w));
    const uint4 r1 = make_uint4((uint32_t)__builtin_amdgcn_ds_bpermute(sl, (int)v1.x),
                                (uint32_t)__builtin_amdgcn_ds_bpermute(sl, (int)v1.y),
                                (uint32_t)__builtin_amdgcn_ds_bpermute(sl, (int)v1.z),
                                (uint32_t)__builtin_amdgcn_ds_bpermute(sl, (int)v1.w));
    return a < (uint32_t)R ? r0 : r1;
}

template <int K, int R = 16, bool FWD = false, bool NT = false, bool DFR = false, bool LA = false>
DEV void row_process(const RowStage<K>& S, uint32_t rl, uint32_t rowbase4, uint8_t* status,
                     nfcs_patch* rec, bool rec_full, bool frame_stores, uint32_t table_n = 0,
                     const uint32_t* wmac = nullptr, const nfcs_nexthop* table = nullptr) {
    const uint32_t len = S.len;
    uint8_t* frame = S.frame;
    const uint4* src = (const uint4*)frame;
    const bool live = S.valid && !S.bad;
    static_assert(K >= 2, "the header view reads slots 0 and 1");
    uint4 h0 = S.v[0];
    if (LA && __builtin_amdgcn_ballot_w64(S.mis != 0) != 0) h0 = hdr_view<K, R>(S, rowbase4, rl);
    bool fwd = false, tagged = false;
    uint32_t fst = NFCS_ST_NONE, ttl = 0, proto = 0;
    if (FWD) {
        const RowHdr<R> h{h0, rowbase4};
        const uint32_t e12 = h.be16(12);
        tagged = e12 == 0x8100u;
        const uint32_t l3t = len < 14 ? 0u : (tagged ? (len >= 18 ? h.be16(16) : e12) : e12);
        const bool v4 = l3t == 0x0800u && (tagged ? 38u : 34u) <= len;
        ttl = tagged ? h.b(26) : h.b(22);
        if (DFR) proto = tagged ? h.b(27) : h.b(23);
        fst = !v4 ? (uint32_t)NFCS_ST_NOT_IPV4
                  : (ttl <= 1 ? (uint32_t)NFCS_ST_TTL_EXPIRED
                              : (S.nh >= table_n ? (uint32_t)NFCS_ST_NO_ROUTE : 0u));
        fwd = live && fst == 0;
        if (fwd && rl == 0 && (!DFR || frame_stores)) {
            constexpr uint32_t PW = 64 / R;
            const uint32_t row = rowbase4 / (4u * R);
            uint32_t m0 = 0, m1 = 0, m2 = 0;
#pragma unroll
            for (uint32_t i = 0; i < PW; ++i) {
                m0 = (row == i) ? wmac[3 * i] : m0;
                m1 = (row == i) ? wmac[3 * i + 1] : m1;
                m2 = (row == i) ? wmac[3 * i + 2] : m2;
            }
            h0.x = m0;
            h0.y = m1;
            h0.z = m2;
        }
        if (fwd && rl == 1) {
            if (tagged) h0.z -= 1u << 16;
            else h0.y -= 1u << 16;
        }
    }
    RPlan P = fast_plan<R, !FWD>(h0, rowbase4, len);
    const bool act = live && (!FWD || fwd);
    const bool slow = act && (P.st >> 8) != 0;
    if (!act || slow)
        P = rplan_none(S.bad ? (uint32_t)NFCS_ST_BAD_DESC
                             : (FWD && live && !fwd) ? fst : (uint32_t)NFCS_ST_NONE);
    const uint32_t st = P.st | ((FWD && fwd) ? (uint32_t)NFCS_ST_FLAG_FWD : 0u);
    const uint32_t ipw = (P.flags & F_IP) ? P.ipw : NFCS_PATCH_NONE;
    uint32_t l4w = NFCS_PATCH_NONE;
    const uint32_t re = (P.flags & F_L4) ? P.re : 0u, lo4 = P.rs & ~3u;
    const uint32_t tailfix = P.flags & F_TAIL;
    uint32_t rlv = rl;
    asm volatile("" : "+v"(rlv));
    uint32_t acc = 0;
    const uint32_t nre = (re + 15u) >> 4;
    {
        const uint32_t last = nre - 1u, la = (!LA || last < (uint32_t)R) ? last : last + S.mis;
        const uint32_t own = (re != 0) && (la < (uint32_t)R * K) && ((la & (R - 1)) == rl);
        uint4 lc = make_uint4(0u, 0u, 0u, 0u);
#pragma unroll
        for (int k = 0; k < K; ++k) {
            const uint4 v = k == 0 ? h0 : S.v[k];
            const uint32_t c = k == 0 ? rlv : rlv + (uint32_t)R * k - S.mis;
            const uint32_t m = (c < nre && (!LA || k != 1 || c >= (uint32_t)R)) ? 0xFFFFFFFFu : 0u;
            if (k == 0) {
                const uint32_t o = 16u * c;
                acc = wsum(v.x & m & ((o >= lo4) ? 0xFFFFFFFFu : 0u), acc);
                acc = wsum(v.y & m & ((o + 4u >= lo4) ? 0xFFFFFFFFu : 0u), acc);
                acc = wsum(v.z & m & ((o + 8u >= lo4) ? 0xFFFFFFFFu : 0u), acc);
                acc = wsum(v.w & m & ((o + 12u >= lo4) ? 0xFFFFFFFFu : 0u), acc);
            } else {
                acc = wsum(v.w & m, wsum(v.z & m, wsum(v.y & m, wsum(v.x & m, acc))));
            }
            const bool sel = (la >> (R == 16 ? 4 : 3)) == (uint32_t)k;
            lc.x = sel ? v.x : lc.x;
            lc.y = sel ? v.y : lc.y;
            lc.z = sel ? v.z : lc.z;
            lc.w = sel ? v.w : lc.w;
        }
        if (own) {
            const uint32_t o = 16u * last, kb8 = 8u * (re - o);
            uint32_t ex = 0;
#pragma unroll
            for (uint32_t j = 0; j < 4; ++j) {
                const int s = min(max((int)kb8 - 32 * (int)j, 0), 32);
                ex = wsum(comp(lc, j) & (uint32_t)(~0ull << s), ex);
            }
            acc -= ex;
            const uint32_t t = re - 1u - o, q = t >> 2;
            const uint32_t dt = q == 0 ? lc.x : (q == 1 ? lc.y : (q == 2 ? lc.z : lc.w));
            if (tailfix) acc += 255u * ((dt >> (8 * (t & 3u))) & 0xFFu);
        }
    }
    const uint32_t cmax = wave_max_rows<R>(LA ? nre + S.mis : nre);
    for (uint32_t cb = (uint32_t)R * K; cb < cmax; cb += (uint32_t)R * K) {
        uint4 w[K];
#pragma unroll
        for (int k = 0; k < K; ++k) {
            const uint32_t c = cb + rlv + (uint32_t)R * k - S.mis;
            w[k] = ld16<1>((c < nre) ? src + c : g_zero_line);
        }
#pragma unroll
        for (int k = 0; k < K; ++k) acc_slot(acc, w[k], cb + rlv + (uint32_t)R * k - S.mis, lo4, re, tailfix);
    }
    const uint32_t z = row_sum<R>(acc) + P.corr;
    if (P.flags & F_L4) {
        uint32_t c = (~fold32(z)) & 0xFFFFu;
        if ((P.flags & F_UDP) && c == 0) c = 0xFFFFu;
        l4w = P.fs | (c << 16);
    }
    const bool ip_new = FWD || (P.old & 0xFFFFu) != (ipw >> 16), l4_new = FWD || (P.old >> 16) != (l4w >> 16);
    const uint32_t sipw = ip_new ? ipw : (uint32_t)NFCS_PATCH_NONE;
    const uint32_t sl4w = l4_new ? l4w : (uint32_t)NFCS_PATCH_NONE;
    auto emit = [&](bool on, uint32_t st_, uint32_t ipw_, uint32_t l4w_, uint32_t sip_, uint32_t sl4_, bool stores,
                    bool recw = true) {
        if (stores && on && rl < 4) {
            const uint32_t w = (rl & 2u) ? sl4_ : sip_;
            const uint32_t pos = (w & 0xFFFFu) + (rl & 1u);
            if ((w & 0xFFFFu) != NFCS_PATCH_NONE) {
                if (NT) st8_nt(frame + pos, w >> (16 + 8 * (rl & 1u)));
                else st8<true>(frame + pos, w >> (16 + 8 * (rl & 1u)));
            }
        }
        if (on && rl == 0) {
            if (status) status[S.p] = (uint8_t)st_;
            if (rec && recw) {
                const uint32_t ri = rec_full ? ipw_ : sip_, rl4 = rec_full ? l4w_ : sl4_;
                uint2 r;
                r.x = (ri & 0xFFFFu) | (rl4 << 16);
                r.y = (ri >> 16) | (rl4 & 0xFFFF0000u);
                ((uint2*)rec)[S.p] = r;
            }
        }
    };
    if (FWD) {
        if (S.valid && !slow && fwd) {
            const uint4 v = put_field(put_field(h0, ipw, rl), l4w, rl);
            uint32_t last = 1u;
            if ((ipw & 0xFFFFu) != NFCS_PATCH_NONE) last = max(last, ((ipw & 0xFFFFu) + 1u) >> 4);
            if ((l4w & 0xFFFFu) != NFCS_PATCH_NONE) last = max(last, ((l4w & 0xFFFFu) + 1u) >> 4);
            if ((!DFR || frame_stores) && rl <= last && 16u * rl < len) {
                if (R == 8 && LA) st16_nt((uint4*)frame + rl, v);
                else st16<true>((uint4*)frame + rl, v);
            }
        }
        emit(S.valid && !slow, st, ipw, l4w, ipw, l4w, false, !DFR);
        if (DFR && rec && S.valid && !slow && rl == 0)
            ((uint2*)rec)[S.p] = (fwd && live) ? fwd_record(ipw, l4w, ttl - 1u, proto, tagged) : make_uint2(0xFFFFFFFFu, 0u);
    } else {
        emit(S.valid && !slow, st, ipw, l4w, sipw, sl4w, frame_stores);
    }
    if (__builtin_amdgcn_ballot_w64(slow) != 0) {
        if (FWD && slow && fwd) {
            if (rl == 0) {
                constexpr uint32_t PW = 64 / R;
                const uint32_t row = rowbase4 / (4u * R);
                uint32_t m[3] = {0, 0, 0};
                if (DFR && !frame_stores) {
#pragma unroll
                    for (uint32_t j = 0; j < 3; ++j) m[j] = ((const uint32_t*)(table + S.nh))[j];
                } else {
#pragma unroll
                    for (uint32_t i = 0; i < PW; ++i) {
#pragma unroll
                        for (uint32_t j = 0; j < 3; ++j) m[j] = (row == i) ? wmac[3 * i + j] : m[j];
                    }
                }
#pragma unroll
                for (uint32_t j = 0; j < 3; ++j)
                    __hip_atomic_store((uint32_t*)frame + j, m[j], __ATOMIC_RELAXED, __HIP_MEMORY_SCOPE_AGENT);
            }
            if (rl == 1) {
                const uint32_t o = tagged ? 26u : 22u;
                st8<true>(frame + o, frame[o] - 1u);
            }
        }
        if (FWD) __builtin_amdgcn_fence(__ATOMIC_SEQ_CST, "agent");
        RPlan Q = rplan_none(0);
        SeqOut o = {0, 0, 0, 0, 0};
        if (slow && rl == 0) {
            Q = slow_plan(frame, len);
            if (Q.flags & F_SEQ) o = seq_update(frame, len);
        }
        Q.st = row_bcast<0, R>(Q.st);
        Q.flags = row_bcast<0, R>(Q.flags);
        Q.ipw = row_bcast<0, R>(Q.ipw);
        Q.rs = row_bcast<0, R>(Q.rs);
        Q.re = row_bcast<0, R>(Q.re);
        Q.fs = row_bcast<0, R>(Q.fs);
        Q.corr = row_bcast<0, R>(Q.corr);
        const uint32_t ost = row_bcast<0, R>(o.st);
        const uint32_t oip = row_bcast<0, R>((o.ip_off & 0xFFFFu) | (o.ip_val << 16));
        const uint32_t ol4 = row_bcast<0, R>((o.l4_off & 0xFFFFu) | (o.l4_val << 16));
        const bool seq = slow && (Q.flags & F_SEQ);
        const uint32_t re2 = (slow && !seq && (Q.flags & F_L4)) ? Q.re : 0u;
        const uint32_t lo42 = Q.rs & ~3u, tf2 = Q.flags & F_TAIL;
        uint32_t acc2 = 0;
        for (uint32_t c = rl; c < ((re2 + 15u) >> 4); c += R) acc_slot(acc2, src[c], c, lo42, re2, tf2);
        const uint32_t z2 = row_sum<R>(acc2) + Q.corr;
        uint32_t st2 = Q.st, ipw2 = (Q.flags & F_IP) ? Q.ipw : NFCS_PATCH_NONE, l4w2 = NFCS_PATCH_NONE;
        if (Q.flags & F_L4) {
            uint32_t c = (~fold32(z2)) & 0xFFFFu;
            if ((Q.flags & F_UDP) && c == 0) c = 0xFFFFu;
            l4w2 = Q.fs | (c << 16);
        }
        if (seq) {
            st2 = ost | NFCS_ST_FLAG_OVERLAP;
            ipw2 = oip;
            l4w2 = ol4;
        }
        if (FWD) st2 |= NFCS_ST_FLAG_FWD;
        emit(slow, st2, ipw2, l4w2, ipw2, l4w2, !seq && (FWD || frame_stores), !(FWD && DFR));
        if (FWD && DFR && rec && slow && rl == 0) ((uint2*)rec)[S.p] = make_uint2(0xFFFFFFFFu, 0u);
    }
}

template <int K, int R, int BS, bool FWD, int SF, bool LA, int PW>
DEV void rows_body(const DescW<PW>& D, uint64_t pw, uint32_t n, uint8_t* arena, uint64_t arena_bytes, uint32_t base16,
                   uint32_t rl, uint32_t row, uint32_t rowbase4, bool defer, const uint32_t (&q)[PW],
                   uint8_t* status, nfcs_patch* patch, nfcs_patch* ws, const nfcs_nexthop* table, uint32_t table_n) {
    typedef const __attribute__((address_space(4))) uint32_t cu32;
    const bool frame_stores = SF == SF_INLINE || (SF == SF_DEFER && !defer);
    nfcs_patch* rec = patch ? patch : (defer ? ws : nullptr);
    RowStage<K> S;
    constexpr bool BUF = !FWD && R == 16 && !LA;
    row_stage<K, R, FWD, LA, BUF>(S, arena, arena_bytes, pick_desc<PW>(D, row), pw + row, n, base16, rl,
                                  wave_buf<PW>(D, pw, n, arena, base16), 0u);
    uint32_t wmac[3 * PW];
    if (FWD) {
#pragma unroll
        for (uint32_t i = 0; i < PW; ++i) S.nh |= (row == i) ? q[i] : 0u;
        if (!(SF == SF_DEFER && defer)) {
#pragma unroll
            for (uint32_t i = 0; i < PW; ++i) {
                const cu32* m = (q[i] < table_n) ? (const cu32*)(table + q[i]) : (const cu32*)g_zero_line;
                wmac[3 * i] = m[0];
                wmac[3 * i + 1] = m[1];
                wmac[3 * i + 2] = m[2];
            }
        }
    }
    row_process<K, R, FWD, !FWD && R == 16 && !LA, FWD && SF == SF_DEFER, LA>(S, rl, rowbase4, status, rec,
                                                                                 patch != nullptr, frame_stores, table_n,
                                                                                 wmac, table);
}

template <int K, int R, int BS, bool FWD, int SF, int LAM, int KL>
DEV void rows_wave(const nfcs_desc* __restrict__ desc, uint32_t n, uint8_t* __restrict__ arena, uint64_t arena_bytes,
                   uint32_t base16, const uint32_t* __restrict__ nh, uint64_t* __restrict__ obs,
                   uint8_t* __restrict__ status, nfcs_patch* __restrict__ patch, nfcs_patch* __restrict__ ws,
                   const nfcs_nexthop* __restrict__ table, uint32_t table_n, uint64_t obs_tag, uint32_t lane,
                   uint32_t rl, uint32_t row, uint32_t rowbase4, uint64_t pw) {
    constexpr uint32_t PW = 64 / R;
    if (blockIdx.x == 0 && threadIdx.x < 64 && obs) sample_footprint(desc, obs_tag, lane, obs);
    const DescW<PW> D = load_descw<PW>(desc, pw, n);
    bool defer = false;
    if (SF == SF_DEFER) {
        static_assert(PW == 4 || PW == 8, "deferral groups of 4 packets");
        uint32_t s0 = 0, s1 = 0;
#pragma unroll
        for (uint32_t i = 0; i < 4; ++i) s0 += defer_len(D.w[2 * i + 1]);
#pragma unroll
        for (uint32_t i = 4; i < PW; ++i) s1 += defer_len(D.w[2 * i + 1]);
        defer = (PW == 8 && row >= 4) ? defer_group(s1, 4) : defer_group(s0, 4);
    }
    typedef const __attribute__((address_space(4))) uint32_t cu32;
    uint32_t q[PW];
    if (FWD) {
        const cu32* nhp = (const cu32*)nh + pw;
        if (pw + PW <= n) {
#pragma unroll
            for (uint32_t i = 0; i < PW; ++i) q[i] = nhp[i];
        } else {
#pragma unroll
            for (uint32_t i = 0; i < PW; ++i) q[i] = (pw + i < n) ? nhp[i] : NFCS_NH_NONE;
        }
    }
    bool la = LAM == 1;
    if (LAM == 2) {
        const nfcs_desc d = pick_desc<PW>(D, row);
        const uint64_t a = (uint64_t)(uintptr_t)arena + ((uint64_t)d.off16 - base16) * 16u;
        la = __builtin_amdgcn_ballot_w64(pw + row < n && d.len != 0 && ((a >> 4) & 7u) != 0) != 0;
    }
    if (la)
        rows_body<KL, R, BS, FWD, SF, true, PW>(D, pw, n, arena, arena_bytes, base16, rl, row, rowbase4, defer, q,
                                                status, patch, ws, table, table_n);
    else
        rows_body<K, R, BS, FWD, SF, false, PW>(D, pw, n, arena, arena_bytes, base16, rl, row, rowbase4, defer, q,
                                                status, patch, ws, table, table_n);
}

template <int K, int R, int OCC, int BS, bool FWD, int SF, int LAM = 0, int KL = K>
__global__ __launch_bounds__(BS, OCC) void update_rows_kernel(const nfcs_desc* __restrict__ desc, uint32_t n,
                                                              uint32_t nblocks, uint8_t* __restrict__ arena,
                                                              uint64_t arena_bytes, uint32_t base16,
                                                              const uint32_t* __restrict__ nh,
                                                              uint64_t* __restrict__ obs,
                                                              uint8_t* __restrict__ status,
                                                              nfcs_patch* __restrict__ patch,
                                                              nfcs_patch* __restrict__ ws,
                                                              const nfcs_nexthop* __restrict__ table,
                                                              uint32_t table_n, uint64_t obs_tag, DoneReq done) {
    constexpr uint32_t PW = 64 / R;
    const uint32_t lane = threadIdx.x & 63u, rl = lane & (R - 1), row = lane / R;
    const uint32_t rowbase4 = (lane & ~(uint32_t)(R - 1)) * 4u;
    const uint64_t pw = (uint64_t)xcd_block_n(nblocks) * (BS / R) + rfl(threadIdx.x >> 6) * PW;
    if (pw >= n && !done.flag) return;
    if (pw < n)
        rows_wave<K, R, BS, FWD, SF, LAM, KL>(desc, n, arena, arena_bytes, base16, nh, obs, status, patch, ws, table,
                                              table_n, obs_tag, lane, rl, row, rowbase4, pw);
    if (done.flag) signal_done(done, nblocks);
}

__global__ __launch_bounds__(kBlock) void apply_bytes_kernel(uint8_t* __restrict__ arena,
                                                             const nfcs_desc* __restrict__ desc,
                                                             uint32_t n, uint32_t base16,
                                                             const nfcs_patch* __restrict__ rec) {
    const uint32_t lane = threadIdx.x & 63u;
    const uint64_t i = (uint64_t)xcd_block() * kBlock + threadIdx.x;
    const nfcs_desc d = i < n ? desc[i] : nfcs_desc{0u, 0u};
    uint2 r0 = make_uint2(0u, 0u);
    if (i < n) r0 = ((const uint2*)rec)[i];
    uint32_t s = defer_len(d.len);
    s += (uint32_t)__builtin_amdgcn_mov_dpp((int)s, 0xB1, 0xF, 0xF, true);
    s += (uint32_t)__builtin_amdgcn_mov_dpp((int)s, 0x4E, 0xF, 0xF, true);
    const bool dfr = i < n && defer_group(s, 4);
    const uint64_t mask = __builtin_amdgcn_ballot_w64(dfr);
    if (!mask) return;
    const uint2 r = dfr ? r0 : make_uint2(NFCS_PATCH_NONE | (NFCS_PATCH_NONE << 16), 0u);
    const uint32_t j = lane & 3u;
#pragma unroll
    for (uint32_t k = 0; k < 4; ++k) {
        if (((mask >> (16u * k)) & 0xFFFFu) == 0) continue;
        const int q4 = (int)((16u * k + (lane >> 2)) * 4u);
        const uint32_t rx = (uint32_t)__builtin_amdgcn_ds_bpermute(q4, (int)r.x);
        const uint32_t ry = (uint32_t)__builtin_amdgcn_ds_bpermute(q4, (int)r.y);
        const uint32_t o16 = (uint32_t)__builtin_amdgcn_ds_bpermute(q4, (int)d.off16);
        const uint32_t ipo = rx & 0xFFFFu, l4o = rx >> 16;
        const uint32_t off = j < 2 ? ipo : l4o;
        const uint32_t a = off + (j & 1u);
        const bool overlap = j < 2 && l4o != NFCS_PATCH_NONE && (a == l4o || a == l4o + 1u);
        if (off != NFCS_PATCH_NONE && !overlap) {
            const uint32_t b = (j < 2 ? (ry >> (8 * j)) : (ry >> (16 + 8 * (j - 2)))) & 0xFFu;
            uint8_t* p = arena + ((uint64_t)o16 - base16) * 16u + a;
            asm volatile("global_store_byte %0, %1, off sc0 sc1 nt" ::"v"(p), "v"(b) : "memory");
        }
    }
}

DEV void st16b_nt(uint8_t* p, uint32_t v) {
    asm volatile("global_store_short %0, %1, off sc0 sc1 nt" ::"v"(p), "v"(v) : "memory");
}

__global__ __launch_bounds__(kBlock) void apply_fwd_kernel(uint8_t* __restrict__ arena,
                                                           const nfcs_desc* __restrict__ desc, uint32_t n,
                                                           const uint32_t* __restrict__ nh,
                                                           const nfcs_nexthop* __restrict__ table,
                                                           const nfcs_patch* __restrict__ rec) {
    const uint32_t lane = threadIdx.x & 63u;
    const uint64_t i = (uint64_t)xcd_block() * kBlock + threadIdx.x;
    const bool in = i < n;
    const nfcs_desc d = in ? desc[i] : nfcs_desc{0u, 0u};
    const uint2 r0 = in ? ((const uint2*)rec)[i] : make_uint2(0xFFFFFFFFu, 0u);
    const uint32_t h = in ? nh[i] : 0u;
    uint32_t s = defer_len(d.len);
    s += (uint32_t)__builtin_amdgcn_mov_dpp((int)s, 0xB1, 0xF, 0xF, true);
    s += (uint32_t)__builtin_amdgcn_mov_dpp((int)s, 0x4E, 0xF, 0xF, true);
    const bool go = in && defer_group(s, 4) && (r0.x & 0xFFu) != kFwdNone;
    const uint64_t mask = __builtin_amdgcn_ballot_w64(go);
    if (!mask) return;
    uint32_t m0 = 0, m1 = 0, m2 = 0;
    if (go) {
        const uint32_t* m = (const uint32_t*)(table + h);
        m0 = m[0];
        m1 = m[1];
        m2 = m[2];
    }
    const uint32_t rx = go ? r0.x : 0xFFFFFFFFu, ry = r0.y;
    const uint32_t j = lane & 15u;
#pragma unroll
    for (uint32_t k = 0; k < 16; ++k) {
        if (((mask >> (4u * k)) & 0xFu) == 0) continue;
        const int q4 = (int)((4u * k + (lane >> 4)) * 4u);
        const uint32_t x = (uint32_t)__builtin_amdgcn_ds_bpermute(q4, (int)rx);
        const uint32_t y = (uint32_t)__builtin_amdgcn_ds_bpermute(q4, (int)ry);
        const uint32_t o16 = (uint32_t)__builtin_amdgcn_ds_bpermute(q4, (int)d.off16);
        const uint32_t a0 = (uint32_t)__builtin_amdgcn_ds_bpermute(q4, (int)m0);
        const uint32_t a1 = (uint32_t)__builtin_amdgcn_ds_bpermute(q4, (int)m1);
        const uint32_t a2 = (uint32_t)__builtin_amdgcn_ds_bpermute(q4, (int)m2);
        const uint32_t ipo = x & 0xFFu, l4o = x >> 24;
        if (ipo == kFwdNone) continue;
        uint8_t* f = arena + (uint64_t)o16 * 16u;
        const uint32_t mw = j < 2 ? a0 : (j < 4 ? a1 : a2);
        uint32_t off = 0xFFFFu, v = 0;
        if (j < 6) {
            off = 2u * j;
            v = mw >> (16u * (j & 1u));
        } else if (j == 6) {
            off = ipo == kFwdNoIp ? (y & 0xFFu) : ipo - 2u;
            v = ((x >> 8) & 0xFFu) | (((x >> 16) & 0xFFu) << 8);
        } else if (j == 7 && ipo != kFwdNoIp) {
            off = ipo;
            v = y;
        } else if (j == 8 && l4o != kFwdNone && !(l4o & 1u)) {
            off = l4o;
            v = y >> 16;
        }
        if (off != 0xFFFFu) st16b_nt(f + off, v & 0xFFFFu);
        if ((j == 8 || j == 9) && l4o != kFwdNone && (l4o & 1u))
            st8_nt(f + l4o + (j - 8u), (y >> (16u + 8u * (j - 8u))) & 0xFFu);
    }
}

enum : int { kShapeTiny = 0, kShapeShort = 1, kShapeLong = 2 };

template <int K, int R, int OCC, int BS, bool FWD, int SF, int LAM = 0, int KL = K>
static void launch_rows(uint32_t grid, unsigned lds, hipStream_t stream, uint8_t* arena, uint64_t arena_bytes,
                        const nfcs_desc* desc, uint32_t n, uint32_t base16, uint8_t* status, nfcs_patch* patch,
                        nfcs_patch* ws, const FwdArgs& fa) {
    hipLaunchKernelGGL((update_rows_kernel<K, R, OCC, BS, FWD, SF, LAM, KL>), dim3(grid), dim3(BS), lds, stream, desc, n, grid,
                       arena, arena_bytes, base16, fa.nh, fa.obs.slot, status, patch, ws, fa.table, fa.table_n,
                       fa.obs.tag, fa.done);
}

static hipError_t launch_update_one(uint8_t* arena, uint64_t arena_bytes, const nfcs_desc* desc, uint32_t n,
                                    uint32_t base16, uint8_t* status, nfcs_patch* patch, nfcs_patch* ws,
                                    int form, int shape, hipStream_t stream, ObsReq obs, DoneReq done = {}) {
    const FwdArgs nofwd = {nullptr, nullptr, 0, obs, done};
    if (form == kUpdateAuto && n <= kInlineMaxPackets) form = kUpdateInline;
    const uint32_t g8 = (n + 7u) / 8u, g4 = (n + 15u) / 16u;
#define NFCS_ROWS(OCC, BS, G, SF)                                                                  \
    launch_rows<6, 16, OCC, BS, false, SF, BS == kBlock ? 1 : 0, BS == kBlock ? 7 : 6>(                          \
        G, BS == kBlock ? kRowsLdsPad : 0u, stream, arena, arena_bytes, desc,                                 \
                                           n, base16, status, patch, ws, nofwd)
#define NFCS_ROWS8(SF) \
    launch_rows<6, 8, 8, 64, false, SF>(g8, 0u, stream, arena, arena_bytes, desc, n, base16, status, patch, ws, nofwd)
#define NFCS_SHORT(SF) \
    launch_rows<6, 16, 7, kBlock, false, SF, 0, 6>(g4, 0u, stream, arena, arena_bytes, desc, n, base16, status, patch, ws, nofwd)
#define NFCS_SHAPED(SF)                                                                            \
    do {                                                                                           \
        if (shape == kShapeTiny) NFCS_ROWS8(SF);                                                   \
        else if (shape == kShapeShort) NFCS_SHORT(SF);                                             \
        else NFCS_ROWS(1, kBlock, g4, SF);                                                         \
    } while (0)
    if (form == kUpdateRecords) {
        NFCS_ROWS(1, kBlock, g4, SF_RECORDS);
    } else if (form == kUpdateInline) {
        NFCS_SHAPED(SF_INLINE);
    } else if (shape != kShapeLong) {
        NFCS_SHAPED(SF_INLINE);
    } else {
        NFCS_ROWS(1, kBlock, g4, SF_DEFER);
        hipLaunchKernelGGL(apply_bytes_kernel, dim3((n + kBlock - 1) / kBlock), dim3(kBlock), 0, stream,
                           arena, desc, n, base16, patch ? patch : ws);
    }
#undef NFCS_SHAPED
#undef NFCS_SHORT
#undef NFCS_ROWS8
#undef NFCS_ROWS
    return hipGetLastError();
}

hipError_t launch_update(const DevInfo& di, uint8_t* arena, uint64_t arena_bytes,
                         const nfcs_desc* desc, uint32_t n, uint32_t base16, uint8_t* status,
                         nfcs_patch* patch, nfcs_patch* ws, int form, hipStream_t stream,
                         uint64_t slot_bytes, ObsReq obs, DoneReq done) {
    (void)di;
    if (n == 0) return hipSuccess;
    if (form == kUpdateRecords && !patch) return hipErrorInvalidValue;
    if (done.flag && form == kUpdateAuto) return hipErrorInvalidValue;
    if (form == kUpdateAuto && !patch && !ws) return hipErrorInvalidValue;
    const uint64_t mean = shape_mean(arena_bytes, n, slot_bytes);
    const int shape = mean < kTinyMeanBytes ? kShapeTiny : (mean < kSmallMeanBytes ? kShapeShort : kShapeLong);
    if (form == kUpdateAuto && shape == kShapeLong && n > kSubBatchAbovePackets) {
        for (uint32_t i = 0; i < n; i += kSubBatchPackets) {
            const hipError_t e = launch_update_one(arena, arena_bytes, desc + i, std::min(kSubBatchPackets, n - i),
                                                   base16, status ? status + i : nullptr,
                                                   patch ? patch + i : nullptr, ws, form, shape, stream,
                                                   i == 0 ? obs : ObsReq{});
            if (e != hipSuccess) return e;
        }
        return hipSuccess;
    }
    return launch_update_one(arena, arena_bytes, desc, n, base16, status, patch, ws, form, shape, stream, obs, done);
}

hipError_t launch_l3_forward(const DevInfo& di, uint8_t* arena, uint64_t arena_bytes,
                             const nfcs_desc* desc, const uint32_t* nh, uint32_t n,
                             const nfcs_nexthop* table, uint32_t table_n, uint8_t* status,
                             nfcs_patch* ws, hipStream_t stream, uint64_t slot_bytes, ObsReq obs) {
    (void)di;
    if (n == 0) return hipSuccess;
    const FwdArgs fa = {nh, table, table_n, obs};
    const uint64_t mean = shape_mean(arena_bytes, n, slot_bytes);
    if (mean < kTinyMeanBytes) {
        launch_rows<6, 8, 8, 64, true, SF_INLINE>((n + 7u) / 8u, 0u, stream, arena, arena_bytes, desc, n, 0u, status,
                                                  nullptr, nullptr, fa);
        return hipGetLastError();
    }
    if (mean < kSmallMeanBytes) {
        launch_rows<12, 8, 6, kBlock, true, SF_INLINE, 1, 12>((n + 31u) / 32u, 0u, stream, arena, arena_bytes, desc, n, 0u, status,
                                                   nullptr, nullptr, fa);
        return hipGetLastError();
    }
    if (ws && n > kFwdDeferAbovePackets) {
        for (uint32_t i = 0; i < n; i += kSubBatchPackets) {
            const uint32_t m = std::min(kSubBatchPackets, n - i);
            const FwdArgs fs = {nh + i, table, table_n, i == 0 ? obs : ObsReq{}};
            launch_rows<6, 16, 7, kBlock, true, SF_DEFER, 2, 7>((m + 15u) / 16u, kRowsLdsPad6, stream, arena, arena_bytes, desc + i, m,
                                                          0u, status ? status + i : nullptr, nullptr, ws, fs);
            hipLaunchKernelGGL(apply_fwd_kernel, dim3((m + kBlock - 1) / kBlock), dim3(kBlock), 0, stream, arena,
                               desc + i, m, nh + i, table, (const nfcs_patch*)ws);
            const hipError_t e = hipGetLastError();
            if (e != hipSuccess) return e;
        }
        return hipSuccess;
    }
    launch_rows<6, 16, 7, kBlock, true, SF_INLINE, 2, 7>((n + 15u) / 16u, 0u, stream, arena, arena_bytes, desc, n, 0u, status,
                                                   nullptr, nullptr, fa);
    return hipGetLastError();
}

enum : uint32_t { VM_NONE = 0, VM_FAIL = 1, VM_RETAG = 2, VM_PUSH = 3, VM_POP = 4 };

DEV uint4 keep_tail(const uint4& nv, const uint4& ov, uint32_t o, uint32_t wend) {
    uint32_t r[4];
#pragma unroll
    for (uint32_t j = 0; j < 4; ++j) {
        const int nb = (int)wend - (int)(o + 4u * j);
        const uint32_t m = nb >= 4 ? 0xFFFFFFFFu : (nb <= 0 ? 0u : ((1u << (8 * nb)) - 1u));
        r[j] = (comp(nv, j) & m) | (comp(ov, j) & ~m);
    }
    return make_uint4(r[0], r[1], r[2], r[3]);
}


DEV uint32_t dpp_prev(uint32_t x) {
    return (uint32_t)__builtin_amdgcn_mov_dpp((int)x, 0x111, 0xF, 0xF, true);
}
DEV uint32_t dpp_next(uint32_t x) {
    return (uint32_t)__builtin_amdgcn_mov_dpp((int)x, 0x101, 0xF, 0xF, true);
}

template <int K, int R = 16>
DEV void vlan_edit(uint4 (&nv)[K], const uint4 (&v)[K], uint32_t mode, uint32_t rl, bool first,
                   uint32_t prevw, uint32_t nextx, uint32_t tag_dw, uint32_t cb, uint32_t wend,
                   uint32_t mis = 0) {
#pragma unroll
    for (int k = 0; k < K; ++k) {
        uint4 e = v[k];
        if (mode == VM_PUSH) {
            uint32_t pw = dpp_prev(v[k].w);
            const uint32_t lw = (k > 0) ? row_bcast<R - 1, R>(v[k - 1].w) : prevw;
            if (rl == 0) pw = lw;
            e = make_uint4(pw, v[k].x, v[k].y, v[k].z);
            if (first && k == 0 && rl == mis) e = make_uint4(v[0].x, v[0].y, v[0].z, tag_dw);
        } else if (mode == VM_POP) {
            uint32_t nx = dpp_next(v[k].x);
            const uint32_t fx = (k + 1 < K) ? row_bcast<0, R>(v[k + 1 < K ? k + 1 : k].x) : nextx;
            if (rl == (uint32_t)R - 1u) nx = fx;
            e = make_uint4(v[k].y, v[k].z, v[k].w, nx);
            if (first && k == 0 && rl == mis) e = make_uint4(v[0].x, v[0].y, v[0].z, nx);
        } else if (mode == VM_RETAG) {
            if (first && k == 0 && rl == mis) e.w = tag_dw;
        }
        const uint32_t c = cb + rl + (uint32_t)R * (uint32_t)k - mis;
        nv[k] = (int)c < 0 ? v[k] : keep_tail(e, v[k], 16u * c, wend);
// ... 1750 lines not shown
    hipLaunchKernelGGL(frames_read_kernel, dim3(grid), dim3(kBlock), kRowsLdsPad, stream, desc, n, grid, arena,
                       arena_bytes, sink);
    return hipGetLastError();
}

uint32_t config_len(int config, uint64_t seed, uint64_t index) { return cfg_len(config, seed, index); }

DEV int hdr_byte(uint32_t o, uint32_t len, uint32_t proto, uint32_t old_ip, uint32_t old_l4) {
    switch (o) {
    case 12: return 0x08;
    case 13: return 0x00;
    case 14: return 0x45;
    case 15: return 0x00;
    case 16: return (int)(((len - 14) >> 8) & 0xFF);
    case 17: return (int)((len - 14) & 0xFF);
    case 22: return 64;
    case 23: return (int)proto;
    case 24: return (int)(old_ip >> 8);
    case 25: return (int)(old_ip & 0xFF);
    default: break;
    }
    if (proto == 17) {
        if (o == 38) return (int)(((len - 34) >> 8) & 0xFF);
        if (o == 39) return (int)((len - 34) & 0xFF);
        if (o == 40) return (int)(old_l4 >> 8);
        if (o == 41) return (int)(old_l4 & 0xFF);
    } else if (proto == 6) {
        if (o == 46) return 0x50;
        if (o == 49) return (int)(old_l4 >> 8);
        if (o == 50) return (int)(old_l4 & 0xFF);
    }
    return -1;
}

__global__ __launch_bounds__(kBlock) void gen_config_kernel(int config, uint64_t seed,
                                                            uint64_t first, uint32_t n,
                                                            uint8_t* __restrict__ arena,
                                                            uint64_t arena_bytes,
                                                            const nfcs_desc* __restrict__ desc) {
    const uint32_t lane = threadIdx.x & 63u;
    const uint32_t nw = gridDim.x * kWavesPerBlock;
    for (uint32_t p = blockIdx.x * kWavesPerBlock + rfl(threadIdx.x >> 6); p < n; p += nw) {
        const nfcs_desc d = desc[p];
        const uint64_t off = (uint64_t)d.off16 * 16u;
        const uint32_t len = d.len;
        if (off + (((uint64_t)len + 15) & ~15ull) > arena_bytes) continue;
        const uint64_t key = pkt_key(seed, first + p);
        const uint32_t proto = config == 0 ? 253u : config == 1 ? 17u : config == 2 ? 6u
                             : ((draw(key, 2) & 1u) ? 6u : 17u);
        const uint32_t old_ip = (uint32_t)((draw(key, 3) & 0xFFFFu) | 0x0101u);
        const uint32_t old_l4 = (uint32_t)((draw(key, 4) & 0xFFFFu) | 0x0101u);
        uint4* dst = (uint4*)(arena + off);
        const uint32_t nch = (len + 15u) >> 4;
        for (uint32_t c = lane; c < nch; c += 64u) {
            uint64_t q[2] = {draw(key, 16 + 2 * c), draw(key, 17 + 2 * c)};
            uint8_t* b = (uint8_t*)q;
            for (uint32_t j = 0; j < 16; ++j) {
                const uint32_t o = c * 16u + j;
                if (o >= len) b[j] = 0;
                else if (o < 64) {
                    int hb = hdr_byte(o, len, proto, old_ip, old_l4);
                    if (hb >= 0) b[j] = (uint8_t)hb;
                }
            }
            uint4 v;
            v.x = (uint32_t)q[0]; v.y = (uint32_t)(q[0] >> 32);
            v.z = (uint32_t)q[1]; v.w = (uint32_t)(q[1] >> 32);
            dst[c] = v;
        }
    }
}

hipError_t launch_gen_config(const DevInfo& di, int config, uint64_t seed, uint64_t first,
                             uint32_t n, uint8_t* arena, uint64_t arena_bytes,
                             const nfcs_desc* desc, hipStream_t stream) {
    if (n == 0) return hipSuccess;
    uint32_t grid = (n + kWavesPerBlock - 1) / kWavesPerBlock;
    if (grid > (uint32_t)di.cus * 8u) grid = (uint32_t)di.cus * 8u;
    hipLaunchKernelGGL(gen_config_kernel, dim3(grid), dim3(kBlock), 0, stream, config, seed,
                       first, n, arena, arena_bytes, desc);
    return hipGetLastError();
}

DEV uint64_t wave_sum64(uint64_t x) {
    uint32_t lo = (uint32_t)x, hi = (uint32_t)(x >> 32);
#define NFCS_DPP_STEP(ctrl)                                                              \
    {                                                                                    \
        uint32_t l2_ = (uint32_t)__builtin_amdgcn_mov_dpp((int)lo, ctrl, 0xF, 0xF, true); \
        uint32_t h2_ = (uint32_t)__builtin_amdgcn_mov_dpp((int)hi, ctrl, 0xF, 0xF, true); \
        uint64_t s_ = ((uint64_t)hi << 32 | lo) + ((uint64_t)h2_ << 32 | l2_);           \
        lo = (uint32_t)s_;                                                               \
        hi = (uint32_t)(s_ >> 32);                                                       \
    }
    NFCS_DPP_STEP(0xB1)
    NFCS_DPP_STEP(0x4E)
    NFCS_DPP_STEP(0x141)
    NFCS_DPP_STEP(0x140)
#undef NFCS_DPP_STEP
    uint64_t s = 0;
#pragma unroll
    for (int r = 0; r < 4; ++r)
        s += ((uint64_t)(uint32_t)__builtin_amdgcn_readlane((int)hi, 16 * r) << 32) |
             (uint32_t)__builtin_amdgcn_readlane((int)lo, 16 * r);
    return s;
}

__global__ __launch_bounds__(kBlock) void digest_kernel(const uint8_t* __restrict__ arena,
                                                        uint64_t arena_bytes,
                                                        const nfcs_desc* __restrict__ desc,
                                                        uint32_t n, uint64_t first,
                                                        unsigned long long* __restrict__ out) {
    const uint32_t lane = threadIdx.x & 63u;
    const uint32_t nw = gridDim.x * kWavesPerBlock;
    uint64_t wsum = 0;
    for (uint32_t p = blockIdx.x * kWavesPerBlock + rfl(threadIdx.x >> 6); p < n; p += nw) {
        const nfcs_desc d = desc[p];
        const uint64_t off = (uint64_t)d.off16 * 16u;
        const uint32_t len = d.len;
        if (off + (((uint64_t)len + 15) & ~15ull) > arena_bytes) continue;
        const uint4* src = (const uint4*)(arena + off);
        const uint32_t nch = (len + 15u) >> 4;
        uint64_t acc = 0;
        for (uint32_t c = lane; c < nch; c += 64u) {
            uint4 v = src[c];
            uint64_t lo = ((uint64_t)v.y << 32) | v.x, hi = ((uint64_t)v.w << 32) | v.z;
            const uint32_t o = c * 16u;
            if (o + 16 > len) {
                const uint32_t keep = len - o;
                if (keep < 8) { lo &= (1ull << (8 * keep)) - 1ull; hi = 0; }
                else if (keep == 8) { hi = 0; }
                else { hi &= (1ull << (8 * (keep - 8))) - 1ull; }
            }
            acc += mix64(lo ^ mix64(hi + (uint64_t)(c + 1) * kGolden));
        }
        const uint64_t h = mix64((uint64_t)len * 0xD6E8FEB86659FD93ull + wave_sum64(acc));
        wsum += mix64(h ^ ((first + p) * 0xA0761D6478BD642Full));
    }
    if (lane == 0 && wsum) atomicAdd(out, (unsigned long long)wsum);
}

hipError_t launch_digest(const DevInfo& di, const uint8_t* arena, uint64_t arena_bytes,
                         const nfcs_desc* desc, uint32_t n, uint64_t first, uint64_t* d_out,
                         hipStream_t stream) {
    if (n == 0) return hipSuccess;
    uint32_t grid = (n + kWavesPerBlock - 1) / kWavesPerBlock;
    if (grid > (uint32_t)di.cus * 8u) grid = (uint32_t)di.cus * 8u;
    hipLaunchKernelGGL(digest_kernel, dim3(grid), dim3(kBlock), 0, stream, arena, arena_bytes,
                       desc, n, first, (unsigned long long*)d_out);
    return hipGetLastError();
}


DEV TxqPort txq_port(const TxqDev& t, uint32_t p) {
    const uint4 r = t.port[p];
    return TxqPort{r.x, r.y, r.z, r.w};
}

DEV uint32_t txq_find_key(const uint32_t* __restrict__ start, uint32_t keys, uint32_t trips, uint32_t e) {
    uint32_t lo = 0, hi = keys + 1u;
    for (uint32_t s = 0; s < trips; ++s) {
        if (lo < hi) {
            const uint32_t mid = (lo + hi) >> 1;
            if (start[mid] > e) hi = mid;
            else lo = mid + 1u;
        }
    }
// ... 169 lines not shown
```

Measured before the change: 6630 GB/s.

## Add adaptive store policy that picks the inline form when few checksums need patching

Sampled workgroups count how many packets actually need a checksum patch. The count goes to a double-buffered device demand array, and the first workgroup of the next launch forwards it to a mapped host word. On the host, a small policy object switches to a sparse (inline) store form after two consecutive low-demand observations. In that form it skips the deferred-records path and the sub-batch split for long packets. The change adds atomics, a cross-launch feedback loop and a test helper kernel that deliberately staleness-corrupts frames. The risk is choosing the wrong form when the data pattern shifts, since the feedback lags by at least one call.

```diff
diff --git a/include/nfcs.h b/include/nfcs.h
--- a/include/nfcs.h
+++ b/include/nfcs.h
@@ -81,6 +81,11 @@
 NFCS_API int nfcs_ctx_set_slot_bytes(nfcs_ctx* ctx, uint32_t bytes);
 NFCS_API int nfcs_ctx_launch_footprint(nfcs_ctx* ctx, uint64_t arena_bytes, const nfcs_desc* d_desc,
                                        uint32_t n, uint64_t* mean);
+#define NFCS_STORE_AUTO 0
+#define NFCS_STORE_DEFERRED 1
+#define NFCS_STORE_SPARSE 2
+NFCS_API int nfcs_ctx_set_store_policy(nfcs_ctx* ctx, int policy);
+NFCS_API int nfcs_ctx_store_state(nfcs_ctx* ctx, int* form, uint32_t* sampled, uint32_t* storing);
 NFCS_API int nfcs_ctx_host_numa(nfcs_ctx* ctx, int* node, int* local);
 
 
@@ -531,6 +536,9 @@
                                     uint64_t first_index, uint32_t n, uint8_t* d_arena,
                                     uint64_t arena_bytes, const nfcs_desc* d_desc, void* stream);
 
+NFCS_API int nfcs_stale_every_device(nfcs_ctx* ctx, uint8_t* d_arena, uint64_t arena_bytes,
+                                     const nfcs_desc* d_desc, uint32_t n, uint32_t every, void* stream);
+
 NFCS_API int nfcs_digest_device(nfcs_ctx* ctx, const uint8_t* d_arena, uint64_t arena_bytes,
                                 const nfcs_desc* d_desc, uint32_t n, uint64_t first_index,
                                 uint64_t* h_digest, void* stream);
diff --git a/netflow_amd/__init__.py b/netflow_amd/__init__.py
--- a/netflow_amd/__init__.py
+++ b/netflow_amd/__init__.py
@@ -96,6 +96,7 @@
 CFG_C0, CFG_C1, CFG_C2, CFG_C3 = 0, 1, 2, 3
 HOST_PATCH_ONLY, HOST_ZERO_COPY, HOST_FRAMES = 1, 2, 4
 PATCH_NONE = 0xFFFF
+STORE_AUTO, STORE_DEFERRED, STORE_SPARSE = 0, 1, 2
 
 
 class NfcsError(RuntimeError):
@@ -132,6 +133,9 @@
         "nfcs_ctx_stream": ([_vp], _vp),
         "nfcs_ctx_set_slot_bytes": ([_vp, ctypes.c_uint32], ctypes.c_int),
         "nfcs_ctx_launch_footprint": ([_vp, _u64, _vp, _u32, ctypes.POINTER(_u64)], ctypes.c_int),
+        "nfcs_ctx_set_store_policy": ([_vp, ctypes.c_int], ctypes.c_int),
+        "nfcs_ctx_store_state": ([_vp, ctypes.POINTER(ctypes.c_int), ctypes.POINTER(_u32), ctypes.POINTER(_u32)],
+                                 ctypes.c_int),
         "nfcs_update_device": ([_vp, _vp, _u64, _vp, _u32, _vp, _vp, _vp], ctypes.c_int),
         "nfcs_update_host": ([_vp, _vp, _u64, _vp, _u32, _vp, _u32], ctypes.c_int),
         "nfcs_update_host_frames": ([_vp, _vp, _vp, _u32, _vp, _u32], ctypes.c_int),
@@ -139,6 +143,7 @@
         "nfcs_shard_bytes": ([_vp, _u32, _u32, _vp], ctypes.c_int),
         "nfcs_ctx_host_numa": ([_vp, ctypes.POINTER(ctypes.c_int), ctypes.POINTER(ctypes.c_int)], ctypes.c_int),
         "nfcs_gen_config_device": ([_vp, ctypes.c_int, _u64, _u64, _u32, _vp, _u64, _vp, _vp], ctypes.c_int),
+        "nfcs_stale_every_device": ([_vp, _vp, _u64, _vp, _u32, _u32, _vp], ctypes.c_int),
         "nfcs_digest_device": ([_vp, _vp, _u64, _vp, _u32, _u64, ctypes.POINTER(_u64), _vp], ctypes.c_int),
         "nfcs_device_alloc": ([_vp, ctypes.c_size_t, ctypes.POINTER(_vp)], ctypes.c_int),
         "nfcs_device_free": ([_vp, _vp], ctypes.c_int),
@@ -916,6 +921,15 @@
         _check(lib().nfcs_ctx_launch_footprint(self.ctx, arena_bytes, p, n, ctypes.byref(m)), "launch_footprint")
         return int(m.value)
 
+    def set_store_policy(self, policy: int):
+        _check(lib().nfcs_ctx_set_store_policy(self.ctx, int(policy)), "set_store_policy")
+
+    def store_state(self) -> tuple[int, int, int]:
+        form, sampled, storing = ctypes.c_int(), _u32(), _u32()
+        _check(lib().nfcs_ctx_store_state(self.ctx, ctypes.byref(form), ctypes.byref(sampled), ctypes.byref(storing)),
+               "store_state")
+        return form.value, int(sampled.value), int(storing.value)
+
     def host_numa(self) -> tuple[int, bool]:
         node, local = ctypes.c_int(), ctypes.c_int()
         _check(lib().nfcs_ctx_host_numa(self.ctx, ctypes.byref(node), ctypes.byref(local)), "host_numa")
@@ -1131,6 +1145,11 @@
         _check(lib().nfcs_gen_config_device(self.ctx, config, seed, first, n, arena.ptr, arena_bytes,
                                             desc.ptr, stream), "gen_config_device")
 
+    def stale_every_device(self, arena: DeviceBuffer, arena_bytes: int, desc: DeviceBuffer, n: int, every: int,
+                           stream=None):
+        _check(lib().nfcs_stale_every_device(self.ctx, arena.ptr, arena_bytes, desc.ptr, n, every, stream),
+               "stale_every_device")
+
     def digest_device(self, arena: DeviceBuffer, arena_bytes: int, desc: DeviceBuffer, n: int,
                       first: int = 0, stream=None) -> int:
         out = _u64()
diff --git a/netflow_amd/csrc/nfcs_api.hip b/netflow_amd/csrc/nfcs_api.hip
--- a/netflow_amd/csrc/nfcs_api.hip
+++ b/netflow_amd/csrc/nfcs_api.hip
@@ -16,6 +16,7 @@
 #include <vector>
 
 #include "nfcs_internal.h"
+#include "nfcs_store_policy.h"
 
 struct HostBlock {
     void* p = nullptr;
@@ -155,6 +156,18 @@
     ObsBurst obs_burst[kObsSlots] = {};
     uint32_t obs_gen = 0;
     uint64_t obs_clock = 0;
+    static constexpr int kDemRing = 64;
+    uint32_t* dem_dev = nullptr;
+    uint64_t* dem_host = nullptr;
+    uint64_t* dem_host_dev = nullptr;
+    uint32_t dem_gen = 0;
+    struct DemCall { uint32_t gen, sampled; };
+    DemCall dem_calls[kDemRing] = {};
+    nfcs::StorePolicy dem_policy;
+    int store_policy = NFCS_STORE_AUTO;
+    int dem_last_form = 0;
+    hipStream_t dem_stream = nullptr;
+    bool dem_any = false;
 };
 
 namespace {
@@ -698,12 +711,45 @@
     return sh;
 }
 
+void read_store_demand(nfcs_ctx* c) {
+    if (!c->dem_host) return;
+    const uint64_t o = __atomic_load_n(c->dem_host, __ATOMIC_RELAXED);
+    const uint32_t gen = (uint32_t)(o >> 32);
+    if (!c->dem_policy.newer(gen)) return;
+    const nfcs_ctx::DemCall& dc = c->dem_calls[gen % nfcs_ctx::kDemRing];
+    if (dc.gen == gen) c->dem_policy.observe(gen, dc.sampled, (uint32_t)o);
+}
+
 int update_device(nfcs_ctx* c, uint8_t* d_arena, uint64_t arena_bytes, const nfcs_desc* d_desc,
                   uint32_t n, uint8_t* d_status, nfcs_patch* d_patch, hipStream_t st) {
     if (!d_patch) NFCS_HIP(acquire_ws(c, n, st));
     const Shape sh = launch_shape(c, arena_bytes, d_desc, n);
+    nfcs::DemandReq dem;
+    bool sparse = false;
+    const bool changed = c->dem_any && c->dem_stream != st;
+    c->dem_stream = st;
+    c->dem_any = true;
+    c->dem_last_form = 0;
+    if (changed) c->dem_policy.reset(c->dem_gen + 2u);
+    if (c->dem_dev && nfcs::update_demand_sampled(arena_bytes, n, sh.mean, false)) {
+        read_store_demand(c);
+        if (!d_patch)
+            sparse = c->store_policy == NFCS_STORE_SPARSE ||
+                     (c->store_policy == NFCS_STORE_AUTO && c->dem_policy.form == nfcs::kStoreFormSparse);
+        const uint32_t prev = c->dem_gen;
+        if (++c->dem_gen == 0) c->dem_gen = 1;
+        const uint32_t words = nfcs::kDemandWords * nfcs::kDemandStrideWords;
+        c->dem_calls[c->dem_gen % nfcs_ctx::kDemRing] = {c->dem_gen,
+                                                         nfcs::update_demand_sampled(arena_bytes, n, sh.mean, sparse)};
+        dem.cur = c->dem_dev + (c->dem_gen & 1u) * words;
+        dem.prev = c->dem_dev + (prev & 1u) * words;
+        dem.host = prev ? c->dem_host_dev : nullptr;
+        dem.prev_gen = prev;
+        if (prev && (prev & 1u) == (c->dem_gen & 1u)) dem.host = nullptr;
+        c->dem_last_form = sparse ? NFCS_STORE_SPARSE : NFCS_STORE_DEFERRED;
+    }
     NFCS_HIP(nfcs::launch_update(c->di, d_arena, arena_bytes, d_desc, n, 0u, d_status, d_patch,
-                                 d_patch ? nullptr : c->ws, nfcs::kUpdateAuto, st, sh.mean, sh.obs));
+                                 d_patch ? nullptr : c->ws, nfcs::kUpdateAuto, st, sh.mean, sh.obs, {}, dem, sparse));
     if (!d_patch) NFCS_HIP(release_ws(c, st));
     return NFCS_OK;
 }
@@ -768,6 +814,14 @@
         for (int k = 0; k < nfcs_ctx::kObsSlots; ++k) c->obs_host[k] = 0;
         e = hipHostGetDevicePointer((void**)&c->obs_dev, c->obs_host, 0);
     }
+    const size_t dem_bytes = 2u * nfcs::kDemandWords * nfcs::kDemandStrideWords * sizeof(uint32_t);
+    if (e == hipSuccess) e = hipMalloc((void**)&c->dem_dev, dem_bytes);
+    if (e == hipSuccess) e = hipMemset(c->dem_dev, 0, dem_bytes);
+    if (e == hipSuccess) e = hipHostMalloc((void**)&c->dem_host, sizeof(uint64_t), hipHostMallocMapped);
+    if (e == hipSuccess) {
+        *c->dem_host = 0;
+        e = hipHostGetDevicePointer((void**)&c->dem_host_dev, c->dem_host, 0);
+    }
     if (e != hipSuccess) {
         nfcs_ctx_destroy(c);
         return hip_fail(e);
@@ -792,6 +846,8 @@
     if (c->ev1) (void)hipEventDestroy(c->ev1);
     if (c->stream) (void)hipStreamDestroy(c->stream);
     if (c->obs_host) (void)hipHostFree(c->obs_host);
+    if (c->dem_host) (void)hipHostFree(c->dem_host);
+    if (c->dem_dev) (void)hipFree(c->dem_dev);
     delete c;
     return NFCS_OK;
 }
@@ -801,6 +857,22 @@
 NFCS_API int nfcs_ctx_set_slot_bytes(nfcs_ctx* c, uint32_t bytes) {
     if (!c) return NFCS_EINVAL;
     c->slot_bytes = bytes;
+    return NFCS_OK;
+}
+
+NFCS_API int nfcs_ctx_set_store_policy(nfcs_ctx* c, int policy) {
+    if (!c || (policy != NFCS_STORE_AUTO && policy != NFCS_STORE_DEFERRED && policy != NFCS_STORE_SPARSE))
+        return NFCS_EINVAL;
+    c->store_policy = policy;
+    return NFCS_OK;
+}
+
+NFCS_API int nfcs_ctx_store_state(nfcs_ctx* c, int* form, uint32_t* sampled, uint32_t* storing) {
+    if (!c) return NFCS_EINVAL;
+    read_store_demand(c);
+    if (form) *form = c->dem_last_form;
+    if (sampled) *sampled = c->dem_policy.obs_sampled;
+    if (storing) *storing = c->dem_policy.obs_storing;
     return NFCS_OK;
 }
 
@@ -2461,6 +2533,17 @@
     return NFCS_OK;
 }
 
+NFCS_API int nfcs_stale_every_device(nfcs_ctx* c, uint8_t* d_arena, uint64_t arena_bytes,
+                                     const nfcs_desc* d_desc, uint32_t n, uint32_t every, void* stream) {
+    if (!c) return NFCS_EINVAL;
+    DeviceGuard dg_(c->di.device);
+    if (dg_.err != hipSuccess) return hip_fail(dg_.err);
+    if (n == 0 || every == 0) return NFCS_OK;
+    if (!d_arena || !d_desc) return NFCS_EINVAL;
+    NFCS_HIP(nfcs::launch_stale_every(d_arena, arena_bytes, d_desc, n, every, pick(c, stream)));
+    return NFCS_OK;
+}
+
 NFCS_API int nfcs_digest_device(nfcs_ctx* c, const uint8_t* d_arena, uint64_t arena_bytes,
                                 const nfcs_desc* d_desc, uint32_t n, uint64_t first,
                                 uint64_t* h_digest, void* stream) {
diff --git a/netflow_amd/csrc/nfcs_internal.h b/netflow_amd/csrc/nfcs_internal.h
--- a/netflow_amd/csrc/nfcs_internal.h
+++ b/netflow_amd/csrc/nfcs_internal.h
@@ -69,10 +69,27 @@
     uint64_t base = 0;
 };
 
+struct DemandReq {
+    uint32_t* cur = nullptr;
+    uint32_t* prev = nullptr;
+    uint64_t* host = nullptr;
+    uint32_t prev_gen = 0;
+};
+constexpr uint32_t kDemandSampleEvery = 64;
+constexpr uint32_t kDemandWords = 64, kDemandStrideWords = 32;
+constexpr uint32_t kDemandBlockPackets = 16;
+inline uint32_t demand_sampled_one(uint32_t n) {
+    const uint32_t span = kDemandSampleEvery * kDemandBlockPackets;
+    const uint32_t rest = n % span;
+    return n / span * kDemandBlockPackets + (rest < kDemandBlockPackets ? rest : kDemandBlockPackets);
+}
+
 hipError_t launch_update(const DevInfo& di, uint8_t* arena, uint64_t arena_bytes,
                          const nfcs_desc* desc, uint32_t n, uint32_t base16, uint8_t* status,
                          nfcs_patch* patch, nfcs_patch* ws, int form, hipStream_t stream,
-                         uint64_t slot_bytes = 0, ObsReq obs = {}, DoneReq done = {});
+                         uint64_t slot_bytes = 0, ObsReq obs = {}, DoneReq done = {}, DemandReq dem = {},
+                         bool sparse = false);
+uint32_t update_demand_sampled(uint64_t arena_bytes, uint32_t n, uint64_t slot_bytes, bool sparse);
 
 hipError_t launch_l3_forward(const DevInfo& di, uint8_t* arena, uint64_t arena_bytes,
                              const nfcs_desc* desc, const uint32_t* nh, uint32_t n,
@@ -230,6 +247,8 @@
 hipError_t launch_icmp_respond(const DevInfo& di, const IcmpView& icmp, const FibView& fib, const IcmpArgs& a,
                                uint32_t* scratch, hipStream_t stream);
 
+hipError_t launch_stale_every(uint8_t* arena, uint64_t arena_bytes, const nfcs_desc* desc, uint32_t n,
+                              uint32_t every, hipStream_t stream);
 hipError_t launch_gen_config(const DevInfo& di, int config, uint64_t seed, uint64_t first,
                              uint32_t n, uint8_t* arena, uint64_t arena_bytes,
                              const nfcs_desc* desc, hipStream_t stream);
diff --git a/netflow_amd/csrc/nfcs_kernels.hip b/netflow_amd/csrc/nfcs_kernels.hip
--- a/netflow_amd/csrc/nfcs_kernels.hip
+++ b/netflow_amd/csrc/nfcs_kernels.hip
@@ -567,6 +567,7 @@
     uint32_t table_n;
     ObsReq obs;
     DoneReq done = {};
+    DemandReq dem = {};
 };
 
 DEV void signal_done(const DoneReq& d, uint32_t nblocks) {
@@ -614,6 +615,18 @@
     if (lane == 0)
         __hip_atomic_store(obs, (tag & 0xFFFFFFFF00000000ull) | kObsPresent | bits | (l << kObsLongShift) | (t >> 8),
                            __ATOMIC_RELAXED, __HIP_MEMORY_SCOPE_SYSTEM);
+}
+
+DEV void forward_demand(const DemandReq& d, uint32_t lane) {
+    static_assert(kDemandWords == 64, "one word per lane");
+    uint32_t* w = d.prev + lane * kDemandStrideWords;
+    uint32_t v = __hip_atomic_load(w, __ATOMIC_RELAXED, __HIP_MEMORY_SCOPE_AGENT);
+    __hip_atomic_store(w, 0u, __ATOMIC_RELAXED, __HIP_MEMORY_SCOPE_AGENT);
+    v = row_sum<16>(v);
+    v = (uint32_t)__builtin_amdgcn_readlane((int)v, 0) + (uint32_t)__builtin_amdgcn_readlane((int)v, 16) +
+        (uint32_t)__builtin_amdgcn_readlane((int)v, 32) + (uint32_t)__builtin_amdgcn_readlane((int)v, 48);
+    if (lane == 0)
+        __hip_atomic_store(d.host, ((uint64_t)d.prev_gen << 32) | v, __ATOMIC_RELAXED, __HIP_MEMORY_SCOPE_SYSTEM);
 }
 
 template <int K, int R = 16, bool FWD = false, bool LA = false, bool BUF = false>
@@ -685,7 +698,8 @@
 template <int K, int R = 16, bool FWD = false, bool NT = false, bool DFR = false, bool LA = false>
 DEV void row_process(const RowStage<K>& S, uint32_t rl, uint32_t rowbase4, uint8_t* status,
                      nfcs_patch* rec, bool rec_full, bool frame_stores, uint32_t table_n = 0,
-                     const uint32_t* wmac = nullptr, const nfcs_nexthop* table = nullptr) {
+                     const uint32_t* wmac = nullptr, const nfcs_nexthop* table = nullptr,
+                     uint32_t* demand = nullptr) {
     const uint32_t len = S.len;
     uint8_t* frame = S.frame;
     const uint4* src = (const uint4*)frame;
@@ -836,6 +850,12 @@
             ((uint2*)rec)[S.p] = (fwd && live) ? fwd_record(ipw, l4w, ttl - 1u, proto, tagged) : make_uint2(0xFFFFFFFFu, 0u);
     } else {
         emit(S.valid && !slow, st, ipw, l4w, sipw, sl4w, frame_stores);
+        if (demand) {
+            const bool need = slow || (sipw & 0xFFFFu) != NFCS_PATCH_NONE || (sl4w & 0xFFFFu) != NFCS_PATCH_NONE;
+            const uint32_t cnt = (uint32_t)__popcll(__builtin_amdgcn_ballot_w64(need && rl == 0));
+            if (cnt != 0 && rl == 0 && rowbase4 == 0)
+                (void)__hip_atomic_fetch_add(demand, cnt, __ATOMIC_RELAXED, __HIP_MEMORY_SCOPE_AGENT);
+        }
     }
     if (__builtin_amdgcn_ballot_w64(slow) != 0) {
         if (FWD && slow && fwd) {
@@ -905,7 +925,8 @@
 template <int K, int R, int BS, bool FWD, int SF, bool LA, int PW>
 DEV void rows_body(const DescW<PW>& D, uint64_t pw, uint32_t n, uint8_t* arena, uint64_t arena_bytes, uint32_t base16,
                    uint32_t rl, uint32_t row, uint32_t rowbase4, bool defer, const uint32_t (&q)[PW],
-                   uint8_t* status, nfcs_patch* patch, nfcs_patch* ws, const nfcs_nexthop* table, uint32_t table_n) {
+                   uint8_t* status, nfcs_patch* patch, nfcs_patch* ws, const nfcs_nexthop* table, uint32_t table_n,
+                   uint32_t* demand) {
     typedef const __attribute__((address_space(4))) uint32_t cu32;
     const bool frame_stores = SF == SF_INLINE || (SF == SF_DEFER && !defer);
     nfcs_patch* rec = patch ? patch : (defer ? ws : nullptr);
@@ -929,7 +950,7 @@
     }
     row_process<K, R, FWD, !FWD && R == 16 && !LA, FWD && SF == SF_DEFER, LA>(S, rl, rowbase4, status, rec,
                                                                                  patch != nullptr, frame_stores, table_n,
-                                                                                 wmac, table);
+                                                                                 wmac, table, demand);
 }
 
 template <int K, int R, int BS, bool FWD, int SF, int LAM, int KL>
@@ -937,7 +958,7 @@
                    uint32_t base16, const uint32_t* __restrict__ nh, uint64_t* __restrict__ obs,
                    uint8_t* __restrict__ status, nfcs_patch* __restrict__ patch, nfcs_patch* __restrict__ ws,
                    const nfcs_nexthop* __restrict__ table, uint32_t table_n, uint64_t obs_tag, uint32_t lane,
-                   uint32_t rl, uint32_t row, uint32_t rowbase4, uint64_t pw) {
+                   uint32_t rl, uint32_t row, uint32_t rowbase4, uint64_t pw, uint32_t* demand) {
     constexpr uint32_t PW = 64 / R;
     if (blockIdx.x == 0 && threadIdx.x < 64 && obs) sample_footprint(desc, obs_tag, lane, obs);
     const DescW<PW> D = load_descw<PW>(desc, pw, n);
@@ -971,10 +992,10 @@
     }
     if (la)
         rows_body<KL, R, BS, FWD, SF, true, PW>(D, pw, n, arena, arena_bytes, base16, rl, row, rowbase4, defer, q,
-                                                status, patch, ws, table, table_n);
+                                                status, patch, ws, table, table_n, demand);
     else
         rows_body<K, R, BS, FWD, SF, false, PW>(D, pw, n, arena, arena_bytes, base16, rl, row, rowbase4, defer, q,
-                                                status, patch, ws, table, table_n);
+                                                status, patch, ws, table, table_n, demand);
 }
 
 template <int K, int R, int OCC, int BS, bool FWD, int SF, int LAM = 0, int KL = K>
@@ -987,15 +1008,25 @@
                                                               nfcs_patch* __restrict__ patch,
                                                               nfcs_patch* __restrict__ ws,
                                                               const nfcs_nexthop* __restrict__ table,
-                                                              uint32_t table_n, uint64_t obs_tag, DoneReq done) {
+                                                              uint32_t table_n, uint64_t obs_tag, DoneReq done,
+                                                              DemandReq dem) {
     constexpr uint32_t PW = 64 / R;
     const uint32_t lane = threadIdx.x & 63u, rl = lane & (R - 1), row = lane / R;
     const uint32_t rowbase4 = (lane & ~(uint32_t)(R - 1)) * 4u;
-    const uint64_t pw = (uint64_t)xcd_block_n(nblocks) * (BS / R) + rfl(threadIdx.x >> 6) * PW;
+    const uint32_t lb = xcd_block_n(nblocks);
+    const uint64_t pw = (uint64_t)lb * (BS / R) + rfl(threadIdx.x >> 6) * PW;
     if (pw >= n && !done.flag) return;
+    constexpr bool DEM = !FWD && R == 16 && LAM == 1 && BS == kBlock && SF != SF_RECORDS;
+    uint32_t* demand = nullptr;
+    if (DEM && dem.cur) {
+        static_assert(!DEM || BS / R == (int)kDemandBlockPackets, "demand_sampled_one counts 16-packet workgroups");
+        if ((lb & (kDemandSampleEvery - 1u)) == 0)
+            demand = dem.cur + ((lb / kDemandSampleEvery) & (kDemandWords - 1u)) * kDemandStrideWords;
+        if (blockIdx.x == 0 && threadIdx.x < 64 && dem.host) forward_demand(dem, lane);
+    }
     if (pw < n)
         rows_wave<K, R, BS, FWD, SF, LAM, KL>(desc, n, arena, arena_bytes, base16, nh, obs, status, patch, ws, table,
-                                              table_n, obs_tag, lane, rl, row, rowbase4, pw);
+                                              table_n, obs_tag, lane, rl, row, rowbase4, pw, demand);
     if (done.flag) signal_done(done, nblocks);
 }
 
@@ -1107,13 +1138,14 @@
                         nfcs_patch* ws, const FwdArgs& fa) {
     hipLaunchKernelGGL((update_rows_kernel<K, R, OCC, BS, FWD, SF, LAM, KL>), dim3(grid), dim3(BS), lds, stream, desc, n, grid,
                        arena, arena_bytes, base16, fa.nh, fa.obs.slot, status, patch, ws, fa.table, fa.table_n,
-                       fa.obs.tag, fa.done);
+                       fa.obs.tag, fa.done, fa.dem);
 }
 
 static hipError_t launch_update_one(uint8_t* arena, uint64_t arena_bytes, const nfcs_desc* desc, uint32_t n,
                                     uint32_t base16, uint8_t* status, nfcs_patch* patch, nfcs_patch* ws,
-                                    int form, int shape, hipStream_t stream, ObsReq obs, DoneReq done = {}) {
-    const FwdArgs nofwd = {nullptr, nullptr, 0, obs, done};
+                                    int form, int shape, hipStream_t stream, ObsReq obs, DoneReq done = {},
+                                    DemandReq dem = {}) {
+    const FwdArgs nofwd = {nullptr, nullptr, 0, obs, done, dem};
     if (form == kUpdateAuto && n <= kInlineMaxPackets) form = kUpdateInline;
     const uint32_t g8 = (n + 7u) / 8u, g4 = (n + 15u) / 16u;
 #define NFCS_ROWS(OCC, BS, G, SF)                                                                  \
@@ -1151,7 +1183,7 @@
 hipError_t launch_update(const DevInfo& di, uint8_t* arena, uint64_t arena_bytes,
                          const nfcs_desc* desc, uint32_t n, uint32_t base16, uint8_t* status,
                          nfcs_patch* patch, nfcs_patch* ws, int form, hipStream_t stream,
-                         uint64_t slot_bytes, ObsReq obs, DoneReq done) {
+                         uint64_t slot_bytes, ObsReq obs, DoneReq done, DemandReq dem, bool sparse) {
     (void)di;
     if (n == 0) return hipSuccess;
     if (form == kUpdateRecords && !patch) return hipErrorInvalidValue;
@@ -1159,17 +1191,28 @@
     if (form == kUpdateAuto && !patch && !ws) return hipErrorInvalidValue;
     const uint64_t mean = shape_mean(arena_bytes, n, slot_bytes);
     const int shape = mean < kTinyMeanBytes ? kShapeTiny : (mean < kSmallMeanBytes ? kShapeShort : kShapeLong);
+    if (form == kUpdateAuto && shape == kShapeLong && sparse && !patch) form = kUpdateInline;
     if (form == kUpdateAuto && shape == kShapeLong && n > kSubBatchAbovePackets) {
         for (uint32_t i = 0; i < n; i += kSubBatchPackets) {
+            const DemandReq ds = {dem.cur, dem.prev, i == 0 ? dem.host : nullptr, dem.prev_gen};
             const hipError_t e = launch_update_one(arena, arena_bytes, desc + i, std::min(kSubBatchPackets, n - i),
                                                    base16, status ? status + i : nullptr,
                                                    patch ? patch + i : nullptr, ws, form, shape, stream,
-                                                   i == 0 ? obs : ObsReq{});
+                                                   i == 0 ? obs : ObsReq{}, DoneReq{}, ds);
             if (e != hipSuccess) return e;
         }
         return hipSuccess;
     }
-    return launch_update_one(arena, arena_bytes, desc, n, base16, status, patch, ws, form, shape, stream, obs, done);
+    return launch_update_one(arena, arena_bytes, desc, n, base16, status, patch, ws, form, shape, stream, obs, done,
+                             dem);
+}
+
+uint32_t update_demand_sampled(uint64_t arena_bytes, uint32_t n, uint64_t slot_bytes, bool sparse) {
+    if (n <= kInlineMaxPackets || shape_mean(arena_bytes, n, slot_bytes) < kSmallMeanBytes) return 0;
+    if (sparse || n <= kSubBatchAbovePackets) return demand_sampled_one(n);
+    uint32_t s = 0;
+    for (uint32_t i = 0; i < n; i += kSubBatchPackets) s += demand_sampled_one(std::min(kSubBatchPackets, n - i));
+    return s;
 }
 
 hipError_t launch_l3_forward(const DevInfo& di, uint8_t* arena, uint64_t arena_bytes,
@@ -3086,6 +3129,32 @@
     return hipGetLastError();
 }
 
+__global__ __launch_bounds__(kBlock) void stale_every_kernel(uint8_t* __restrict__ arena, uint64_t arena_bytes,
+                                                             const nfcs_desc* __restrict__ desc, uint32_t n,
+                                                             uint32_t every) {
+    const uint64_t g = (uint64_t)blockIdx.x * kBlock + threadIdx.x;
+    uint32_t h = (uint32_t)g * 0x9E3779B1u;
+    h ^= h >> 15;
+    h *= 0x85EBCA77u;
+    h ^= h >> 13;
+    const uint64_t p = g * every + h % every;
+    if (p >= n) return;
+    const nfcs_desc d = desc[p];
+    const uint64_t off = (uint64_t)d.off16 * 16u;
+    if (d.len < 42u || off + (((uint64_t)d.len + 15u) & ~15ull) > arena_bytes) return;
+    arena[off + 24u] ^= 0xFFu;
+    arena[off + 40u] ^= 0xFFu;
+}
+
+hipError_t launch_stale_every(uint8_t* arena, uint64_t arena_bytes, const nfcs_desc* desc, uint32_t n,
+                              uint32_t every, hipStream_t stream) {
+    if (n == 0 || every == 0) return hipSuccess;
+    const uint32_t m = (n + every - 1u) / every;
+    hipLaunchKernelGGL(stale_every_kernel, dim3((m + kBlock - 1u) / kBlock), dim3(kBlock), 0, stream, arena,
+                       arena_bytes, desc, n, every);
+    return hipGetLastError();
+}
+
 DEV uint64_t wave_sum64(uint64_t x) {
     uint32_t lo = (uint32_t)x, hi = (uint32_t)(x >> 32);
 #define NFCS_DPP_STEP(ctrl)                                                              \
diff --git a/netflow_amd/csrc/nfcs_store_policy.h b/netflow_amd/csrc/nfcs_store_policy.h
--- /dev/null
+++ b/netflow_amd/csrc/nfcs_store_policy.h
@@ -0,0 +1,44 @@
+#pragma once
+#include <cstdint>
+
+namespace nfcs {
+
+enum : int { kStoreFormDeferred = 0, kStoreFormSparse = 1 };
+
+constexpr uint32_t kSparseMaxNum = 1, kSparseMaxDen = 512;
+constexpr uint32_t kSparseLowRun = 2;
+
+struct StorePolicy {
+    int form = kStoreFormDeferred;
+    uint32_t last_gen = 0;
+    uint32_t low_run = 0;
+    uint32_t obs_gen = 0, obs_sampled = 0, obs_storing = 0;
+
+    static bool low(uint32_t sampled, uint32_t storing) {
+        return (uint64_t)storing * kSparseMaxDen < (uint64_t)sampled * kSparseMaxNum;
+    }
+    bool newer(uint32_t gen) const { return gen != 0 && (int32_t)(gen - last_gen) > 0; }
+
+    void observe(uint32_t gen, uint32_t sampled, uint32_t storing) {
+        if (!newer(gen) || sampled == 0) return;
+        last_gen = gen;
+        obs_gen = gen;
+        obs_sampled = sampled;
+        obs_storing = storing < sampled ? storing : sampled;
+        if (low(sampled, storing)) {
+            if (low_run < kSparseLowRun) ++low_run;
+            if (low_run >= kSparseLowRun) form = kStoreFormSparse;
+        } else {
+            low_run = 0;
+            form = kStoreFormDeferred;
+        }
+    }
+    void reset(uint32_t ignore_through) {
+        form = kStoreFormDeferred;
+        low_run = 0;
+        last_gen = ignore_through;
+        obs_gen = obs_sampled = obs_storing = 0;
+    }
+};
+
+}
```

After: 6824 GB/s, median of 6. 2.9% higher.
